# vimalabs/VIMA

Measured on NVIDIA B200. Metric: policy steps/sec (batched action decode), higher is better.
Workload: dtype f16 hi*hi + e4m3 cross terms (2 tensor pass-equivalents), f16 3-term in attention, fp32 accumulate/softmax/LN

## Files before the change

### vima_b200/build.py

```python
from __future__ import annotations

import hashlib
import os
import subprocess
import sys
from concurrent.futures import ThreadPoolExecutor

HERE = os.path.dirname(os.path.abspath(__file__))
CSRC = os.path.join(HERE, "csrc")
OUT_DIR = os.path.join(HERE, "_lib")
LIB_PATH = os.path.join(OUT_DIR, "libvima_b200.so")
SOURCES = ["api.cu", "gemm_tc_f16.cu", "gemm_tc_bf16.cu", "norm.cu", "attention.cu", "attention_tc.cu", "attention_tail.cu", "gemm_simt.cu", "misc.cu", "prepare.cu"]
HEADERS = ["common.cuh", "kernels.h", "gemm_tc.cuh", "gemm_tc_variants.cuh", os.path.join("..", "..", "include", "vima_b200.h")]
NVCC_FLAGS = [
    "-gencode", "arch=compute_100a,code=sm_100a", "-O3", "-lineinfo", "-std=c++17", "--expt-relaxed-constexpr",
    "-Xcompiler", "-fPIC", "-Xcompiler", "-fvisibility=hidden",
]


def _nvcc() -> str:
    for p in (os.environ.get("NVCC"), "/usr/local/cuda/bin/nvcc", "nvcc"):
        if p and (os.path.isfile(p) or p == "nvcc"):
            return p
    raise RuntimeError("nvcc not found")


def _digest() -> str:
    h = hashlib.sha256()
    for f in SOURCES + HEADERS:
        with open(os.path.join(CSRC, f), "rb") as fh:
            h.update(fh.read())
    h.update(" ".join(NVCC_FLAGS).encode())
    return h.hexdigest()


def build(force: bool = False, verbose: bool = False) -> str:
    os.makedirs(OUT_DIR, exist_ok=True)
    stamp = os.path.join(OUT_DIR, "build.sha256")
    dig = _digest()
    if not force and os.path.isfile(LIB_PATH) and os.path.isfile(stamp) and open(stamp).read().strip() == dig:
        return LIB_PATH
    nvcc = _nvcc()

    def compile_one(src: str) -> str:
        obj = os.path.join(OUT_DIR, src.replace(".cu", ".o"))
        cmd = [nvcc, *NVCC_FLAGS, "-c", os.path.join(CSRC, src), "-o", obj]
        if verbose:
            cmd.insert(1, "-Xptxas")
            cmd.insert(2, "-v")
        r = subprocess.run(cmd, capture_output=True, text=True)
        if r.returncode != 0:
            raise RuntimeError(f"nvcc failed for {src}:\n{r.stdout}\n{r.stderr}")
        if verbose:
            print(r.stderr)
        return obj

    with ThreadPoolExecutor(max_workers=len(SOURCES)) as ex:
        objs = list(ex.map(compile_one, SOURCES))
    r = subprocess.run([nvcc, "-shared", "-o", LIB_PATH, *objs, "-cudart", "static"], capture_output=True, text=True)
    if r.returncode != 0:
        raise RuntimeError(f"link failed:\n{r.stdout}\n{r.stderr}")
    with open(stamp, "w") as fh:
        fh.write(dig)
    return LIB_PATH


if __name__ == "__main__":
    print(build(force="--force" in sys.argv, verbose="--verbose" in sys.argv))
```

### vima_b200/csrc/api.cu

```cuda
#include <cstdarg>
#include <cstddef>
#include <cstdio>
#include <cstring>
#include <cstdlib>

#include "../../include/vima_b200.h"
#include "gemm_tc_variants.cuh"
#include "kernels.h"

using namespace vima;

struct vima_ctx {
  int device;
  int sm_count;
  int max_smem_optin;
  long long launches;
  char err[512];
  void* encode_tiled;
  bool gemm_attr_set;
  int attn_tc;
  int attn_tail;
  int gemm_mode;
  int epi_prefetch;
};

struct DeviceGuard {
  int prev = -1;
  bool armed = false;
  cudaError_t enter(int dev) {
    cudaError_t e = cudaGetDevice(&prev);
    if (e != cudaSuccess) return e;
    if (prev == dev) return cudaSuccess;
    armed = true;
    return cudaSetDevice(dev);
  }
  ~DeviceGuard() {
    if (armed) cudaSetDevice(prev);
  }
};

typedef CUresult (*PFN_encodeTiled)(CUtensorMap*, CUtensorMapDataType, cuuint32_t, void*, const cuuint64_t*, const cuuint64_t*,
                                    const cuuint32_t*, const cuuint32_t*, CUtensorMapInterleave, CUtensorMapSwizzle,
                                    CUtensorMapL2promotion, CUtensorMapFloatOOBfill);

static int fail(vima_ctx* c, int code, const char* fmt, ...) {
  if (c) {
    va_list ap;
    va_start(ap, fmt);
    vsnprintf(c->err, sizeof(c->err), fmt, ap);
    va_end(ap);
  }
  return code;
}
static int cuda_fail(vima_ctx* c, cudaError_t e, const char* what) {
  return fail(c, VIMA_E_CUDA, "%s: %s", what, cudaGetErrorString(e));
}
#define CHECK_CTX(c)                  \
  if (!(c)) return VIMA_E_INVALID;    \
  DeviceGuard dev_guard_;             \
  {                                   \
    cudaError_t e_ = dev_guard_.enter((c)->device); \
    if (e_ != cudaSuccess) return cuda_fail((c), e_, "cudaSetDevice"); \
  }

template <class D>
static int load_desc(vima_ctx* c, const D* in, D* out, size_t min_size, const char* what) {
  if (!in) return fail(c, VIMA_E_INVALID, "%s: null descriptor", what);
  const uint32_t sz = in->struct_size;
  if (sz < min_size || sz > sizeof(D))
    return fail(c, VIMA_E_INVALID, "%s: descriptor struct_size %u outside [%zu, %zu] (C-ABI v%d): the caller was built against another vima_b200.h",
                what, sz, min_size, sizeof(D), VIMA_B200_ABI_VERSION);
  memset(out, 0, sizeof(D));
  memcpy(out, in, sz);
  return VIMA_OK;
}
#define LAUNCHED(c, expr, name)                          \
  {                                                      \
    cudaError_t e_ = (expr);                             \
    if (e_ != cudaSuccess) return cuda_fail((c), e_, name); \
    (c)->launches++;                                     \
    return VIMA_OK;                                      \
  }

extern "C" {

int vima_abi_version(void) { return VIMA_B200_ABI_VERSION; }

int vima_set_option(vima_ctx* c, const char* key, const char* value) {
  if (!c) return VIMA_E_INVALID;
  if (!key || !value) return fail(c, VIMA_E_INVALID, "set_option: null key or value");
  if (!strcmp(key, "attn")) {
    if (!strcmp(value, "tc")) { c->attn_tc = 1; return VIMA_OK; }
    if (!strcmp(value, "mma")) { c->attn_tc = 0; return VIMA_OK; }
  } else if (!strcmp(key, "attn_tail")) {
    if (!strcmp(value, "kernel")) { c->attn_tail = 1; return VIMA_OK; }
    if (!strcmp(value, "off")) { c->attn_tail = 0; return VIMA_OK; }
  } else if (!strcmp(key, "gemm_mode")) {
    if (!strcmp(value, "1cta")) { c->gemm_mode = 0; return VIMA_OK; }
    if (!strcmp(value, "mcast")) { c->gemm_mode = 1; return VIMA_OK; }
    if (!strcmp(value, "2cta")) { c->gemm_mode = 2; return VIMA_OK; }
  } else if (!strcmp(key, "epi_prefetch")) {
    if (!strcmp(value, "0") || !strcmp(value, "1")) { c->epi_prefetch = value[0] == '1'; return VIMA_OK; }
  }
  return fail(c, VIMA_E_INVALID, "set_option: unknown option %s=%s", key, value);
}

int vima_create(vima_ctx** out, int device) {
  if (!out) return VIMA_E_INVALID;
  *out = nullptr;
  int n = 0;
  if (cudaGetDeviceCount(&n) != cudaSuccess || device < 0 || device >= n) return VIMA_E_CUDA;
  cudaDeviceProp prop;
  if (cudaGetDeviceProperties(&prop, device) != cudaSuccess) return VIMA_E_CUDA;
  if (prop.major != 10) return VIMA_E_UNSUPPORTED;
  vima_ctx* c = new vima_ctx();
  memset(c, 0, sizeof(*c));
  c->device = device;
  c->sm_count = prop.multiProcessorCount;
  c->max_smem_optin = (int)prop.sharedMemPerBlockOptin;
  DeviceGuard guard;
  if (guard.enter(device) != cudaSuccess) { delete c; return VIMA_E_CUDA; }
  cudaFree(0);
  cudaDriverEntryPointQueryResult q;
  void* fn = nullptr;
  if (cudaGetDriverEntryPoint("cuTensorMapEncodeTiled", &fn, cudaEnableDefault, &q) != cudaSuccess || fn == nullptr) {
    delete c;
    return VIMA_E_CUDA;
  }
  c->encode_tiled = fn;
  c->attn_tc = 1; c->attn_tail = 1; c->gemm_mode = 2; c->epi_prefetch = 0;
  if (const char* e = getenv("VIMA_B200_ATTN")) vima_set_option(c, "attn", e);
  if (const char* e = getenv("VIMA_B200_ATTN_TAIL")) vima_set_option(c, "attn_tail", e);
  if (const char* e = getenv("VIMA_B200_GEMM_MODE")) vima_set_option(c, "gemm_mode", e);
  if (const char* e = getenv("VIMA_B200_EPI_PREFETCH")) vima_set_option(c, "epi_prefetch", e);
  c->err[0] = 0;
  *out = c;
  return VIMA_OK;
}

void vima_destroy(vima_ctx* c) { delete c; }
const char* vima_last_error(vima_ctx* c) { return c ? c->err : "null context"; }
int vima_sm_count(vima_ctx* c) { return c ? c->sm_count : 0; }
int vima_sizeof_gemm_desc(void) { return (int)sizeof(vima_gemm_desc); }
int vima_sizeof_norm_desc(void) { return (int)sizeof(vima_norm_desc); }
int vima_sizeof_attn_desc(void) { return (int)sizeof(vima_attn_desc); }
int vima_sizeof_f32_gemm_group(void) { return (int)sizeof(vima_f32_gemm_group); }
int64_t vima_launch_count(vima_ctx* c) { return c ? c->launches : 0; }

int vima_split_f32(vima_ctx* c, const float* x, int64_t rows, int cols, int ldx, void* hi, void* lo, int ld16, int pad_cols, float scale,
                   int dtype, void* stream) {
  CHECK_CTX(c);
  if (!x || !hi || pad_cols < cols || pad_cols > ld16) return fail(c, VIMA_E_INVALID, "split_f32: bad arguments");
  LAUNCHED(c, launch_split(x, rows, cols, ldx, (unsigned short*)hi, (unsigned short*)lo, ld16, pad_cols, scale, dtype, (cudaStream_t)stream),
           "split_f32");
}

int vima_pack_weight(vima_ctx* c, const float* w, int n, int k, int transposed, int ldw, void* hi, void* lo, int ld16, float scale, int dtype,
                     void* stream) {
  CHECK_CTX(c);
  if (!w || !hi || ld16 < k || (ld16 & 7)) return fail(c, VIMA_E_INVALID, "pack_weight: ld16 must be >= k and a multiple of 8");
  LAUNCHED(c, launch_pack_weight(w, n, k, transposed, ldw, (unsigned short*)hi, (unsigned short*)lo, ld16, scale, dtype, (cudaStream_t)stream),
           "pack_weight");
}

int vima_pack_weight_f8(vima_ctx* c, const float* w, int n, int k, int transposed, int ldw, void* hi8, void* lo8, int ld8, float scale, void* stream) {
  CHECK_CTX(c);
  if (!w || !hi8 || !lo8 || ld8 < k || (ld8 & 15)) return fail(c, VIMA_E_INVALID, "pack_weight_f8: ld8 must be >= k and a multiple of 16");
  LAUNCHED(c, launch_pack_weight_f8(w, n, k, transposed, ldw, (unsigned char*)hi8, (unsigned char*)lo8, ld8, scale, (cudaStream_t)stream),
           "pack_weight_f8");
}

int vima_split_f8(vima_ctx* c, const float* x, int64_t rows, int cols, int ldx, void* lo8, void* hi8, int ld8, void* stream) {
  CHECK_CTX(c);
  if (!x || !lo8 || !hi8 || (cols & 3) || (ldx & 3) || (ld8 & 3) || ld8 < cols) return fail(c, VIMA_E_INVALID, "split_f8: bad arguments");
  LAUNCHED(c, launch_split_f8(x, rows, cols, ldx, (unsigned char*)lo8, (unsigned char*)hi8, ld8, (cudaStream_t)stream), "split_f8");
}

static int choose_block_n(int N, int glu) {
  const int step = glu ? 64 : 32;
  int best = step, best_pad = 1 << 30;
  for (int bn = step; bn <= 256; bn += step) {
    const int padded = ((N + bn - 1) / bn) * bn;
    if (padded < best_pad || (padded == best_pad && bn > best)) { best = bn; best_pad = padded; }
  }
  return best;
}
int vima_glu_block_n(int n_out) { return choose_block_n(2 * n_out, 1); }
int vima_gemm_stats_parts(int N, int glu, int block_n) {
  const int bn = block_n > 0 ? block_n : choose_block_n(N, glu);
  return 2 * ((N + bn - 1) / bn);
}

int vima_row_stats_finalize(vima_ctx* c, const float* partial, int64_t rows, int parts, int cols, float eps, int rms, float* stats, void* stream) {
  CHECK_CTX(c);
  if (!partial || !stats || rows < 0 || parts <= 0 || cols <= 0 || ((uintptr_t)partial & 7) || ((uintptr_t)stats & 7))
    return fail(c, VIMA_E_INVALID, "row_stats_finalize: bad arguments");
  LAUNCHED(c, launch_row_stats_finalize(partial, rows, parts, cols, eps, rms, stats, (cudaStream_t)stream), "row_stats_finalize");
}

static int make_tmap_f8(vima_ctx* c, CUtensorMap* tm, const void* base, int rows, int cols, int ld, int box_rows) {
  const cuuint64_t gdim[2] = {(cuuint64_t)cols, (cuuint64_t)rows};
  const cuuint64_t gstride[1] = {(cuuint64_t)ld};
  const cuuint32_t box[2] = {(cuuint32_t)GEMM_BK, (cuuint32_t)box_rows};
  const cuuint32_t estr[2] = {1, 1};
  CUresult r = ((PFN_encodeTiled)c->encode_tiled)(tm, CU_TENSOR_MAP_DATA_TYPE_UINT8, 2, const_cast<void*>(base), gdim, gstride, box, estr,
                                                  CU_TENSOR_MAP_INTERLEAVE_NONE, CU_TENSOR_MAP_SWIZZLE_64B, CU_TENSOR_MAP_L2_PROMOTION_L2_256B,
                                                  CU_TENSOR_MAP_FLOAT_OOB_FILL_NONE);
  if (r != CUDA_SUCCESS) return fail(c, VIMA_E_CUDA, "cuTensorMapEncodeTiled(fp8) failed (%d): rows %d cols %d ld %d box %d", (int)r, rows, cols, ld, box_rows);
  return VIMA_OK;
}

static int make_tmap(vima_ctx* c, CUtensorMap* tm, const void* base, int dtype, int rows, int cols, int ld, int box_rows) {
  const cuuint64_t gdim[2] = {(cuuint64_t)cols, (cuuint64_t)rows};
  const cuuint64_t gstride[1] = {(cuuint64_t)ld * 2};
  const cuuint32_t box[2] = {(cuuint32_t)GEMM_BK, (cuuint32_t)box_rows};
  const cuuint32_t estr[2] = {1, 1};
  const CUtensorMapDataType dt = dtype == DT_BF16 ? CU_TENSOR_MAP_DATA_TYPE_BFLOAT16 : CU_TENSOR_MAP_DATA_TYPE_FLOAT16;
  CUresult r = ((PFN_encodeTiled)c->encode_tiled)(tm, dt, 2, const_cast<void*>(base), gdim, gstride, box, estr, CU_TENSOR_MAP_INTERLEAVE_NONE,
                                                  CU_TENSOR_MAP_SWIZZLE_128B, CU_TENSOR_MAP_L2_PROMOTION_L2_256B,
                                                  CU_TENSOR_MAP_FLOAT_OOB_FILL_NONE);
  if (r != CUDA_SUCCESS) return fail(c, VIMA_E_CUDA, "cuTensorMapEncodeTiled failed (%d): rows %d cols %d ld %d box %d", (int)r, rows, cols, ld, box_rows);
  return VIMA_OK;
}

int vima_gemm(vima_ctx* c, const vima_gemm_desc* d_in, void* stream) {
  CHECK_CTX(c);
  vima_gemm_desc d_local;
  if (int rc_ = load_desc(c, d_in, &d_local, VIMA_GEMM_DESC_V4_SIZE, "gemm")) return rc_;
  const vima_gemm_desc* d = &d_local;
  if (!d->a_hi || !d->b_hi) return fail(c, VIMA_E_INVALID, "gemm: null operand");
  if (d->M <= 0 || d->N <= 0 || d->K <= 0) return fail(c, VIMA_E_INVALID, "gemm: empty problem");
  if ((d->lda & 7) || (d->ldb & 7) || ((uintptr_t)d->a_hi & 15) || ((uintptr_t)d->b_hi & 15))
    return fail(c, VIMA_E_INVALID, "gemm: operands need 16-byte aligned bases and ld %% 8 == 0 (lda %d ldb %d)", d->lda, d->ldb);
  if ((d->a_lo == nullptr) != (d->b_lo == nullptr)) return fail(c, VIMA_E_INVALID, "gemm: a_lo and b_lo must both be set or both be null");
  const bool f8 = d->a_lo8 || d->a_hi8 || d->b_hi8 || d->b_lo8;
  if (f8) {
    if (!(d->a_lo8 && d->a_hi8 && d->b_hi8 && d->b_lo8) || d->a_lo || d->dtype != DT_F16)
      return fail(c, VIMA_E_INVALID, "gemm: f16f8 mode needs all four e4m3 operands, fp16 hi operands and no 16-bit lo operands");
    if ((d->lda8 & 15) || (d->ldb8 & 15) || ((uintptr_t)d->a_lo8 & 15) || ((uintptr_t)d->a_hi8 & 15) || ((uintptr_t)d->b_hi8 & 15) ||
        ((uintptr_t)d->b_lo8 & 15) || d->lda8 < d->K || d->ldb8 < d->K)
      return fail(c, VIMA_E_INVALID, "gemm: e4m3 operands need 16-byte aligned bases and ld %% 16 == 0");
  }
  if ((d->out_lo8 == nullptr) != (d->out_hi8 == nullptr) || (d->out_lo8 && (!d->out_hi || d->dtype != DT_F16 || (d->ld_o8 & 3))))
    return fail(c, VIMA_E_INVALID, "gemm: out_lo8/out_hi8 come together, with an fp16 out_hi, ld_o8 %% 4 == 0");
  if (d->lda < d->K || d->ldb < d->K) return fail(c, VIMA_E_INVALID, "gemm: leading dimension smaller than K");
  int bn = d->block_n > 0 ? d->block_n : choose_block_n(d->N, d->glu);
  if (bn > 256 || (bn % (d->glu ? 64 : 32))) return fail(c, VIMA_E_INVALID, "gemm: bad block_n %d", bn);
  if (d->glu && (d->N % bn)) return fail(c, VIMA_E_INVALID, "gemm: GLU needs N %% block_n == 0");
  {
    const int n_out = d->glu ? d->N / 2 : d->N;
    const bool bad = (n_out & 3) || (d->out_f32 && ((d->ld_o32 & 3) || ((uintptr_t)d->out_f32 & 15))) ||
                     (d->out_hi && ((d->ld_o16 & 3) || ((uintptr_t)d->out_hi & 7) || (d->out_lo && ((uintptr_t)d->out_lo & 7)))) ||
                     (d->mul && ((d->ld_mul & 3) || ((uintptr_t)d->mul & 15))) || (d->residual && ((d->ld_res & 3) || ((uintptr_t)d->residual & 15)));
    if (bad) return fail(c, VIMA_E_INVALID, "gemm: epilogue tensors need N %% 4 == 0, ld %% 4 == 0 and 16-byte (fp32) / 8-byte (16-bit) aligned bases");
  }

  if (d->row_stats) {
    if (!d->ln_c1 || (d->ln_cols != 1 && d->ln_cols != 2) || (d->ln_cols == 2 && !d->glu) || ((uintptr_t)d->row_stats & 7))
      return fail(c, VIMA_E_INVALID, "gemm: folded LayerNorm needs row_stats (8-byte aligned), ln_c1 and ln_cols 1 (all columns) or 2 (GLU value half)");
  }
  if (d->res_stats) {
    if (!d->residual || !d->res_gamma || !d->res_beta || d->glu || ((uintptr_t)d->res_stats & 7))
      return fail(c, VIMA_E_INVALID, "gemm: a LayerNorm'd residual needs residual, res_stats (8-byte aligned), res_gamma, res_beta and no GLU");
  }
  if (d->stats_out) {
    if (d->stats_parts != 2 * ((d->N + bn - 1) / bn) || ((uintptr_t)d->stats_out & 7))
      return fail(c, VIMA_E_INVALID, "gemm: stats_parts must be vima_gemm_stats_parts(N, glu, block_n) = %d (got %d)", 2 * ((d->N + bn - 1) / bn), d->stats_parts);
  }

  GemmParams p;
  memset(&p, 0, sizeof(p));
  const int split = f8 ? 2 : (d->a_lo != nullptr ? 1 : 0);
  int rc;
  const int tiles_m_ = (d->M + GEMM_BM - 1) / GEMM_BM, tiles_n_ = (d->N + bn - 1) / bn;
  const int mode_pref = c->gemm_mode;
  const bool pair_ok = (bn % 64) == 0 && ((tiles_m_ + 1) / 2) * tiles_n_ >= c->sm_count / 2 && tiles_m_ >= 2;
  const int mcast = (pair_ok && mode_pref == 1) ? 1 : 0;
  const int two_cta = (pair_ok && mode_pref == 2) ? 1 : 0;
  const int b_box = (mcast || two_cta) ? bn / 2 : bn;
  if ((rc = make_tmap(c, &p.tm_a_hi, d->a_hi, d->dtype, d->M, d->K, d->lda, GEMM_BM))) return rc;
  if ((rc = make_tmap(c, &p.tm_b_hi, d->b_hi, d->dtype, d->N, d->K, d->ldb, b_box))) return rc;
  if (split == 1) {
    if ((rc = make_tmap(c, &p.tm_a_lo, d->a_lo, d->dtype, d->M, d->K, d->lda, GEMM_BM))) return rc;
    if ((rc = make_tmap(c, &p.tm_b_lo, d->b_lo, d->dtype, d->N, d->K, d->ldb, b_box))) return rc;
  } else if (split == 2) {
    if ((rc = make_tmap_f8(c, &p.tm_a_lo, d->a_lo8, d->M, d->K, d->lda8, GEMM_BM))) return rc;
    if ((rc = make_tmap_f8(c, &p.tm_a_hi8, d->a_hi8, d->M, d->K, d->lda8, GEMM_BM))) return rc;
    if ((rc = make_tmap_f8(c, &p.tm_b_hi8, d->b_hi8, d->N, d->K, d->ldb8, b_box))) return rc;
    if ((rc = make_tmap_f8(c, &p.tm_b_lo, d->b_lo8, d->N, d->K, d->ldb8, b_box))) return rc;
  }
  p.M = d->M; p.N = d->N; p.K = d->K;
  p.block_n = bn;
  p.mcast = mcast;
  p.two_cta = two_cta;
  p.split = split;
  p.dtype = d->dtype;
  p.glu = d->glu;
  p.epi_prefetch = c->epi_prefetch;
  p.act = d->act;
  p.acc_scale = d->acc_scale == 0.f ? 1.f : d->acc_scale;
  p.bias = d->bias;
  p.mul = d->mul; p.ld_mul = d->ld_mul;
  p.residual = d->residual; p.ld_res = d->ld_res;
  p.out_f32 = d->out_f32; p.ld_o32 = d->ld_o32;
  p.out_hi = (unsigned short*)d->out_hi; p.out_lo = (unsigned short*)d->out_lo; p.ld_o16 = d->ld_o16;
  p.out_lo8 = (unsigned char*)d->out_lo8; p.out_hi8 = (unsigned char*)d->out_hi8; p.ld_o8 = d->ld_o8;
  p.row_stats = d->row_stats; p.ln_c1 = d->ln_c1; p.ln_cols = d->ln_cols;
  p.res_stats = d->res_stats; p.res_gamma = d->res_gamma; p.res_beta = d->res_beta;
  p.stats_out = d->stats_out; p.stats_parts = d->stats_parts;

  const size_t stage = (size_t)(GEMM_A_TILE_BYTES + (two_cta ? bn / 2 : bn) * 128) * (split ? 2 : 1);
  const size_t fixed = gemm_smem_bytes(bn, split, 0, two_cta);
  int n_stages = (int)(((size_t)c->max_smem_optin - fixed) / stage);
  if (n_stages > GEMM_MAX_STAGES) n_stages = GEMM_MAX_STAGES;
  if (n_stages < 2) return fail(c, VIMA_E_UNSUPPORTED, "gemm: not enough shared memory for 2 stages");
  p.n_stages = n_stages;
  const size_t smem = gemm_smem_bytes(bn, split, n_stages, two_cta);
  const int tiles = mcast ? ((tiles_m_ + 1) / 2) * tiles_n_ : tiles_m_ * tiles_n_;
  int grid = tiles < c->sm_count ? tiles : c->sm_count;
  if (mcast || two_cta) grid = 2 * (tiles < c->sm_count / 2 ? tiles : c->sm_count / 2);
  GemmLaunch l;
  l.act = d->act; l.glu = d->glu != 0; l.mul = d->mul != nullptr; l.res = d->residual != nullptr;
  l.o32 = d->out_f32 != nullptr; l.o16 = d->out_hi != nullptr; l.dtype = d->dtype;
  l.lna = d->row_stats != nullptr; l.lnr = d->res_stats != nullptr; l.stats = d->stats_out != nullptr; l.device = c->device;
  if (d->dtype == DT_BF16) { LAUNCHED(c, launch_gemm_tc_bf16(p, l, grid, smem, c->max_smem_optin, (cudaStream_t)stream), "gemm_tc_kernel"); }
  LAUNCHED(c, launch_gemm_tc_f16(p, l, grid, smem, c->max_smem_optin, (cudaStream_t)stream), "gemm_tc_kernel");
}

int vima_gemm_f32_grouped(vima_ctx* c, const vima_f32_gemm_group* groups_dev, int n_groups, int M, int max_n, int act, void* stream) {
  CHECK_CTX(c);
  static_assert(sizeof(vima_f32_gemm_group) == sizeof(SimtGemmGroup), "group layout");
  if (!groups_dev) return fail(c, VIMA_E_INVALID, "gemm_f32_grouped: null groups");
  LAUNCHED(c, launch_simt_gemm_grouped(reinterpret_cast<const SimtGemmGroup*>(groups_dev), n_groups, M, max_n, act, (cudaStream_t)stream),
           "simt_gemm");
}

int vima_gemm_f32_grouped_host(vima_ctx* c, const vima_f32_gemm_group* groups_host, int n_groups, int M, int max_n, int act, void* stream) {
  CHECK_CTX(c);
  if (!groups_host || n_groups < 0) return fail(c, VIMA_E_INVALID, "gemm_f32_grouped_host: null groups");
  cudaError_t e = launch_simt_gemm_grouped_host(reinterpret_cast<const SimtGemmGroup*>(groups_host), n_groups, M, max_n, act, (cudaStream_t)stream);
  if (e != cudaSuccess) return cuda_fail(c, e, "simt_gemm");
  c->launches += (n_groups + SIMT_MAX_HOST_GROUPS - 1) / SIMT_MAX_HOST_GROUPS;
  return VIMA_OK;
}

int vima_norm(vima_ctx* c, const vima_norm_desc* d_in, void* stream) {
  CHECK_CTX(c);
  vima_norm_desc d_local;
  if (int rc_ = load_desc(c, d_in, &d_local, VIMA_NORM_DESC_V4_SIZE, "norm")) return rc_;
  const vima_norm_desc* d = &d_local;
  if (!d->x) return fail(c, VIMA_E_INVALID, "norm: null input");
  if ((d->cols & 3) || d->cols > 1024 || d->cols <= 0) return fail(c, VIMA_E_INVALID, "norm: cols must be a multiple of 4, <= 1024 (got %d)", d->cols);
  if ((d->ldx & 3) || (d->add && (d->ld_add & 3)) || (d->out_f32 && (d->ld_o32 & 3)) || (d->out2_f32 && (d->ld_o2 & 3)) || (d->out_hi && (d->ld_o16 & 3)))
    return fail(c, VIMA_E_INVALID, "norm: leading dimensions must be multiples of 4");
  NormParams p;
  p.x = d->x; p.rows = d->rows; p.cols = d->cols; p.ldx = d->ldx;
  p.add = d->add; p.ld_add = d->ld_add;
  p.w = d->w; p.b = d->b; p.eps = d->eps; p.rms = d->rms;
  p.w2 = d->w2; p.b2 = d->b2; p.eps2 = d->eps2;
  p.out_f32 = d->out_f32; p.ld_o32 = d->ld_o32;
  p.out2_f32 = d->out2_f32; p.ld_o2 = d->ld_o2;
  p.out_hi = (unsigned short*)d->out_hi; p.out_lo = (unsigned short*)d->out_lo; p.ld_o16 = d->ld_o16;
  p.dtype = d->dtype;
  p.out_lo8 = (unsigned char*)d->out_lo8; p.out_hi8 = (unsigned char*)d->out_hi8; p.ld_o8 = d->ld_o8;
  p.stats_out = d->stats_out; p.stats_eps = d->stats_eps;
  if (p.stats_out && ((uintptr_t)p.stats_out & 7)) return fail(c, VIMA_E_INVALID, "norm: stats_out must be 8-byte aligned");
  if ((p.out_lo8 == nullptr) != (p.out_hi8 == nullptr) || (p.out_lo8 && (p.ld_o8 & 3)))
    return fail(c, VIMA_E_INVALID, "norm: out_lo8/out_hi8 come together with ld_o8 %% 4 == 0");
  LAUNCHED(c, launch_norm(p, (cudaStream_t)stream), "norm");
}

int vima_attention(vima_ctx* c, const vima_attn_desc* d_in, void* stream) {
  CHECK_CTX(c);
  vima_attn_desc d_local;
  if (int rc_ = load_desc(c, d_in, &d_local, VIMA_ATTN_DESC_V4_SIZE, "attention")) return rc_;
  const vima_attn_desc* d = &d_local;
  if (!d->q_hi || !d->k_hi || !d->v_hi || !d->o_hi) return fail(c, VIMA_E_INVALID, "attention: null operand");
  if (d->D != 32 && d->D != 64) return fail(c, VIMA_E_UNSUPPORTED, "attention: head_dim %d (32 and 64 are built)", d->D);
  if ((d->ldq & 7) || (d->ldk & 7) || (d->ldv & 7) || (d->ldo & 1)) return fail(c, VIMA_E_INVALID, "attention: leading dimensions must be multiples of 8");
  const bool split = d->q_lo != nullptr;
  if (split != (d->k_lo != nullptr) || split != (d->v_lo != nullptr)) return fail(c, VIMA_E_INVALID, "attention: q/k/v lo parts must be all set or all null");
  if (d->rel_bias && d->Lq != d->Lk) return fail(c, VIMA_E_INVALID, "attention: relative bias needs Lq == Lk");
  if (!(d->scale > 0.f)) return fail(c, VIMA_E_INVALID, "attention: scale must be positive");
  AttnParams p;
  p.q_hi = (const unsigned short*)d->q_hi; p.q_lo = (const unsigned short*)d->q_lo; p.ldq = d->ldq;
  p.k_hi = (const unsigned short*)d->k_hi; p.k_lo = (const unsigned short*)d->k_lo; p.ldk = d->ldk;
  p.v_hi = (const unsigned short*)d->v_hi; p.v_lo = (const unsigned short*)d->v_lo; p.ldv = d->ldv;
  p.key_mask = d->key_mask; p.rel_bias = d->rel_bias;
  p.o_hi = (unsigned short*)d->o_hi; p.o_lo = (unsigned short*)d->o_lo; p.ldo = d->ldo;
  p.B = d->B; p.H = d->H; p.Lq = d->Lq; p.Lk = d->Lk; p.D = d->D;
  p.scale = d->scale; p.causal = d->causal; p.split = split; p.dtype = d->dtype;
  p.o_lo8 = (unsigned char*)d->o_lo8; p.o_hi8 = (unsigned char*)d->o_hi8; p.ldo8 = d->ldo8;
  p.kv_batch_rows = d->kv_batch_rows; p.mask_ld = d->mask_ld; p.q_pos0 = d->q_pos0; p.q_batch_rows = 0;
  if ((d->kv_batch_rows && d->kv_batch_rows < d->Lk) || (d->mask_ld && d->mask_ld < d->Lk) || d->q_pos0 < 0)
    return fail(c, VIMA_E_INVALID, "attention: kv_batch_rows / mask_ld must cover Lk, q_pos0 >= 0");
  if ((p.o_lo8 == nullptr) != (p.o_hi8 == nullptr) || (p.o_lo8 && ((p.ldo8 & 1) || d->dtype != DT_F16)))
    return fail(c, VIMA_E_INVALID, "attention: o_lo8/o_hi8 come together (fp16 format, even ldo8)");
  if (c->attn_tc && attention_tc_supported(p)) {
    const int tail = p.Lq % 128;
    if (c->attn_tail && p.Lq > 128 && tail >= 1 && tail <= ATTN_TAIL_MAX_ROWS) {
      AttnParams body = p;
      body.Lq = p.Lq - tail;
      body.q_batch_rows = p.Lq;
      cudaError_t e_ = launch_attention_tc(body, c->encode_tiled, (cudaStream_t)stream);
      if (e_ != cudaSuccess) return cuda_fail(c, e_, "attention_tc");
      c->launches++;
      LAUNCHED(c, launch_attention_tail(p, p.Lq - tail, tail, (cudaStream_t)stream), "attention_tail");
    }
    LAUNCHED(c, launch_attention_tc(p, c->encode_tiled, (cudaStream_t)stream), "attention_tc");
  }
  {
    const size_t need = attention_smem_bytes(p);
    if (need > (size_t)c->max_smem_optin)
      return fail(c, VIMA_E_UNSUPPORTED,
                  "attention: Lk = %d keys of head_dim %d (%s operands%s) need %zu bytes of shared memory, the device offers %d: the "
                  "resident-K/V kernel takes Lk <= %d at this head_dim", d->Lk, d->D, split ? "split" : "single", d->rel_bias ? ", relative bias" : "",
                  need, c->max_smem_optin, attention_max_lk(p, (size_t)c->max_smem_optin));
  }
  LAUNCHED(c, launch_attention(p, (cudaStream_t)stream), "attention");
}

int vima_latent_attention(vima_ctx* c, const float* q, int ldq, int64_t q_batch_stride, const float* k, int ldk, const float* v, int ldv, float* o,
                          int ldo, int64_t N, int Lq, int Lk, int H, int d, float scale, void* stream) {
  CHECK_CTX(c);
  if (!q || !k || !v || !o) return fail(c, VIMA_E_INVALID, "latent_attention: null pointer");
  if (Lk < 1 || Lk > 16 || d < 1 || d > 128 || Lq < 0 || N < 0 || H < 1)
    return fail(c, VIMA_E_UNSUPPORTED, "latent_attention: 1..16 keys, head_dim <= 128 (Lk %d, d %d)", Lk, d);
  LatentAttnParams p;
  p.q = q; p.ldq = ldq; p.q_batch_stride = q_batch_stride; p.k = k; p.ldk = ldk; p.v = v; p.ldv = ldv; p.o = o; p.ldo = ldo;
  p.N = N; p.Lq = Lq; p.Lk = Lk; p.H = H; p.d = d; p.scale = scale;
  LAUNCHED(c, launch_latent_attention(p, (cudaStream_t)stream), "latent_attention");
}

int vima_small_attention(vima_ctx* c, const float* qkv, int ld, int64_t N, int S, int H, int W, float scale, void* o_hi, void* o_lo, int ldo,
                         float* o_f32, int dtype, void* stream) {
  CHECK_CTX(c);
  if (!qkv) return fail(c, VIMA_E_INVALID, "small_attention: null input");
  SmallAttnParams p;
  p.qkv = qkv; p.ld = ld; p.o_hi = (unsigned short*)o_hi; p.o_lo = (unsigned short*)o_lo; p.ldo = ldo; p.o_f32 = o_f32;
  p.N = N; p.S = S; p.H = H; p.W = W; p.scale = scale; p.dtype = dtype;
  LAUNCHED(c, launch_small_attention(p, (cudaStream_t)stream), "small_attention");
}

int vima_assemble_history(vima_ctx* c, const float* obs, const uint8_t* obs_mask, const float* action, int T, int B, int Q, int E, int La,
                          float* tokens, uint8_t* masks_bl, int64_t* pos_bl, void* stream) {
  CHECK_CTX(c);
  if (!obs || !obs_mask || !tokens || !masks_bl || !pos_bl || (La > 0 && !action) || (E & 3))
    return fail(c, VIMA_E_INVALID, "assemble_history: bad arguments");
  if (La != T && La != T - 1) return fail(c, VIMA_E_INVALID, "assemble_history: need T-1 or T action tokens");
  cudaError_t e = launch_assemble_history(obs, obs_mask, action, T, B, Q, E, La, tokens, masks_bl, (long long*)pos_bl, (cudaStream_t)stream);
  if (e != cudaSuccess) return cuda_fail(c, e, "assemble_history");
  c->launches += 2;
  return VIMA_OK;
}

int vima_mask_cumsum(vima_ctx* c, const uint8_t* mask, int B, int L, int64_t* pos, void* stream) {
  CHECK_CTX(c);
  LAUNCHED(c, launch_mask_cumsum(mask, B, L, (long long*)pos, (cudaStream_t)stream), "mask_cumsum");
}

int vima_add_pos_embed(vima_ctx* c, const float* tok, int64_t stride_b, int64_t stride_l, const int64_t* ids, const float* table, int n_pos, int B,
                       int L, int E, float* out_f32, void* hi, void* lo, int ld16, int dtype, int* err_flag, void* stream) {
  CHECK_CTX(c);
  if ((E & 3) || (stride_b & 3) || (stride_l & 3) || (hi && (ld16 & 3))) return fail(c, VIMA_E_INVALID, "add_pos_embed: alignment");
  LAUNCHED(c, launch_add_pos_embed(tok, stride_b, stride_l, (const long long*)ids, table, n_pos, B, L, E, out_f32, (unsigned short*)hi,
                                   (unsigned short*)lo, ld16, dtype, err_flag, (cudaStream_t)stream),
           "add_pos_embed");
}

int vima_gather_prompt(vima_ctx* c, const int32_t* kind, const int32_t* index, const int64_t* word_ids, const float* word_table,
                       const float* img_emb, const uint8_t* img_mask, int B, int Lp, int D, float* out, uint8_t* mask_out, void* stream) {
  CHECK_CTX(c);
  if (D & 3) return fail(c, VIMA_E_INVALID, "gather_prompt: D %% 4");
  LAUNCHED(c, launch_gather_prompt(kind, index, (const long long*)word_ids, word_table, img_emb, img_mask, B, Lp, D, out, mask_out,
                                   (cudaStream_t)stream),
           "gather_prompt");
}

int vima_patchify(vima_ctx* c, const uint8_t* img, int64_t N, int H, int W, int P, void* hi, void* lo, int ld16, int dtype, void* stream) {
  CHECK_CTX(c);
  if ((P & 3) || (H % P) || (W % P) || (ld16 & 3) || ld16 < 3 * P * P) return fail(c, VIMA_E_INVALID, "patchify: bad geometry");
  LAUNCHED(c, launch_patchify(img, N, H, W, P, (unsigned short*)hi, (unsigned short*)lo, ld16, dtype, (cudaStream_t)stream), "patchify");
}

int vima_vit_tokens(vima_ctx* c, const float* patch_out, const float* cls, const float* pos, int64_t N, int S, int W, float* out, void* stream) {
  CHECK_CTX(c);
  if (W & 3) return fail(c, VIMA_E_INVALID, "vit_tokens: W %% 4");
  LAUNCHED(c, launch_vit_tokens(patch_out, cls, pos, N, S, W, out, (cudaStream_t)stream), "vit_tokens");
}

int vima_bbox_norm(vima_ctx* c, const int64_t* bbox, int64_t n, float* out, void* stream) {
  CHECK_CTX(c);
  LAUNCHED(c, launch_bbox_norm((const long long*)bbox, n, out, (cudaStream_t)stream), "bbox_norm");
}

int vima_fill_ee(vima_ctx* c, const int64_t* ee, const float* table, int64_t n_te, int Q, void* hi, void* lo, int ld16, int col0, int n_pad,
                 int dtype, void* stream) {
  CHECK_CTX(c);
  LAUNCHED(c, launch_fill_ee((const long long*)ee, table, n_te, Q, (unsigned short*)hi, (unsigned short*)lo, ld16, col0, n_pad, dtype,
                             (cudaStream_t)stream),
           "fill_ee");
}

int vima_gato_positions(vima_ctx* c, const uint8_t* prompt_mask, int B, int Lp, int L, uint8_t* mask_out, int64_t* pos_out, void* stream) {
  CHECK_CTX(c);
  if (!prompt_mask || !mask_out || !pos_out || L < Lp) return fail(c, VIMA_E_INVALID, "gato_positions: bad arguments");
  LAUNCHED(c, launch_gato_positions(prompt_mask, B, Lp, L, mask_out, (long long*)pos_out, (cudaStream_t)stream), "gato_positions");
}

int vima_max_u8(vima_ctx* c, const uint8_t* x, int64_t n, int* out_max, void* stream) {
  CHECK_CTX(c);
  LAUNCHED(c, launch_max_u8(x, n, out_max, (cudaStream_t)stream), "max_u8");
}

int vima_action_scale(vima_ctx* c, const int64_t* idx, int64_t n, int width, const float* bins_dev, float* out, void* stream) {
  CHECK_CTX(c);
  LAUNCHED(c, launch_action_scale((const long long*)idx, n, width, bins_dev, out, (cudaStream_t)stream), "action_scale");
}

int vima_object_stats(vima_ctx* c, const void* segm, int segm_elem_bytes, int n_img, int H, int W, const int64_t* obj_ids_dev, int n_obj,
                      int ids_per_image, int32_t* stats, void* stream) {
  CHECK_CTX(c);
  if ((segm_elem_bytes != 1 && segm_elem_bytes != 4 && segm_elem_bytes != 8) || n_obj < 0 || n_obj > 64 || n_img < 0 || H <= 0 || W <= 0)
    return fail(c, VIMA_E_INVALID, "object_stats: segm elements of 1/4/8 bytes, at most 64 object ids per image");
  LAUNCHED(c, launch_object_stats(segm, segm_elem_bytes, n_img, H, W, (const long long*)obj_ids_dev, n_obj, ids_per_image, stats,
                                  (cudaStream_t)stream), "object_stats");
}

int vima_crop_resize(vima_ctx* c, const uint8_t* rgb, int n_img, int H, int W, const int32_t* stats, int n_obj, uint8_t* crops,
                     int64_t* bbox, uint8_t* mask, int32_t* n_valid, void* stream) {
  CHECK_CTX(c);
  if (n_obj < 0 || n_obj > 64 || n_img < 0 || n_img > 65535 || H <= 0 || W <= 0)
    return fail(c, VIMA_E_INVALID, "crop_resize: at most 64 object ids per image and 65535 images per call");
  LAUNCHED(c, launch_crop_resize(rgb, n_img, H, W, stats, n_obj, crops, (long long*)bbox, mask, n_valid, (cudaStream_t)stream),
           "crop_resize");
}

int vima_action_postprocess(vima_ctx* c, const int64_t* idx, int64_t n, int width, const float* bins_dev, const float* lo_dev,
                            const float* hi_dev, int bound_stride, float* out, void* stream) {
  CHECK_CTX(c);
  if (width <= 0 || n < 0 || (bound_stride != 0 && bound_stride < width))
    return fail(c, VIMA_E_INVALID, "action_postprocess: width > 0, n >= 0, bound_stride 0 (broadcast) or >= width");
  LAUNCHED(c, launch_action_post((const long long*)idx, n, width, bins_dev, lo_dev, hi_dev, bound_stride, out, (cudaStream_t)stream),
           "action_postprocess");
}

int vima_head_select(vima_ctx* c, const float* logits, int B, int n_heads, const int32_t* head_off_dev, float* logits_norm, int64_t* modes,
                     void* stream) {
  CHECK_CTX(c);
  LAUNCHED(c, launch_head_select(logits, B, n_heads, head_off_dev, logits_norm, (long long*)modes, (cudaStream_t)stream), "head_select");
}

}
```

### vima_b200/csrc/attention.cu

```cuda
#include "kernels.h"

namespace vima {

constexpr float FP32_MIN = -3.4028234663852886e38f;
constexpr float LOG2E = 1.4426950408889634f;

template <int DT>
__device__ __forceinline__ void mma16816(float (&c)[4], const uint32_t (&a)[4], uint32_t b0, uint32_t b1) {
  if constexpr (DT == DT_F16) {
    asm volatile("mma.sync.aligned.m16n8k16.row.col.f32.f16.f16.f32 {%0,%1,%2,%3}, {%4,%5,%6,%7}, {%8,%9}, {%0,%1,%2,%3};"
                 : "+f"(c[0]), "+f"(c[1]), "+f"(c[2]), "+f"(c[3])
                 : "r"(a[0]), "r"(a[1]), "r"(a[2]), "r"(a[3]), "r"(b0), "r"(b1));
  } else {
    asm volatile("mma.sync.aligned.m16n8k16.row.col.f32.bf16.bf16.f32 {%0,%1,%2,%3}, {%4,%5,%6,%7}, {%8,%9}, {%0,%1,%2,%3};"
                 : "+f"(c[0]), "+f"(c[1]), "+f"(c[2]), "+f"(c[3])
                 : "r"(a[0]), "r"(a[1]), "r"(a[2]), "r"(a[3]), "r"(b0), "r"(b1));
  }
}

template <int DT>
__device__ __forceinline__ void pack_split(float x0, float x1, uint32_t& hi, uint32_t& lo) { split2<DT>(x0, x1, hi, lo); }

__device__ __forceinline__ void ldmatrix_x4(uint32_t (&r)[4], const void* smem_row_ptr) {
  asm volatile("ldmatrix.sync.aligned.m8n8.x4.shared.b16 {%0,%1,%2,%3}, [%4];"
               : "=r"(r[0]), "=r"(r[1]), "=r"(r[2]), "=r"(r[3])
               : "r"(smem_u32(smem_row_ptr)));
}

constexpr float CAUSAL_L2 = -1e4f * LOG2E;
constexpr float EXIT_L2 = -9000.f * LOG2E;

template <int D, int DT, bool SPLIT>
__global__ void __launch_bounds__(256, (D == 32) ? 2 : 1) attention_kernel(const AttnParams p) {
  constexpr int KS = D / 16;
  constexpr int ND = D / 8;
  constexpr int KROW = D + 8;
  extern __shared__ __align__(16) unsigned char smem[];
  const int h = blockIdx.x, b = blockIdx.y;
  const int Lk = p.Lk, Lq = p.Lq;
  const int Lk_pad = (Lk + 63) & ~63;
  const int VROW = Lk_pad + 8;
  const int n_kt = Lk_pad / 64;
  unsigned short* Ks_hi = reinterpret_cast<unsigned short*>(smem);
  unsigned short* Ks_lo = Ks_hi + (SPLIT ? Lk_pad * KROW : 0);
  unsigned short* Vt_hi = Ks_lo + Lk_pad * KROW;
  unsigned short* Vt_lo = Vt_hi + (SPLIT ? D * VROW : 0);
  float* maskadd = reinterpret_cast<float*>(Vt_lo + D * VROW);
  int* tile_plain = reinterpret_cast<int*>(maskadd + Lk_pad);
  int* qb_counter = tile_plain + n_kt;
  float* sbias = reinterpret_cast<float*>(qb_counter + 1);

  const int tid = threadIdx.x, lane = tid & 31, warp = tid >> 5;
  const int kvb = p.kv_batch_rows ? p.kv_batch_rows : Lk;
  const int mld = p.mask_ld ? p.mask_ld : Lk;
  const int qp0 = p.q_pos0;
  const int qbr = p.q_batch_rows ? p.q_batch_rows : Lq;
  constexpr int CH = D / 8;
  for (int idx = tid; idx < Lk_pad * CH; idx += 256) {
    const int j = idx / CH, c = idx % CH;
    uint4 kh = make_uint4(0, 0, 0, 0), kl = kh, vh = kh, vl = kh;
    if (j < Lk) {
      const size_t rk = ((size_t)b * kvb + j) * p.ldk + h * D + c * 8;
      const size_t rv = ((size_t)b * kvb + j) * p.ldv + h * D + c * 8;
      kh = __ldg(reinterpret_cast<const uint4*>(p.k_hi + rk));
      vh = __ldg(reinterpret_cast<const uint4*>(p.v_hi + rv));
      if (SPLIT) {
        kl = __ldg(reinterpret_cast<const uint4*>(p.k_lo + rk));
        vl = __ldg(reinterpret_cast<const uint4*>(p.v_lo + rv));
      }
    }
    *reinterpret_cast<uint4*>(Ks_hi + j * KROW + c * 8) = kh;
    if (SPLIT) *reinterpret_cast<uint4*>(Ks_lo + j * KROW + c * 8) = kl;
    const unsigned short* vhs = reinterpret_cast<const unsigned short*>(&vh);
    const unsigned short* vls = reinterpret_cast<const unsigned short*>(&vl);
#pragma unroll
    for (int e = 0; e < 8; ++e) {
      Vt_hi[(c * 8 + e) * VROW + j] = vhs[e];
      if (SPLIT) Vt_lo[(c * 8 + e) * VROW + j] = vls[e];
    }
  }
  for (int j = tid; j < Lk_pad; j += 256) {
    float m = -INFINITY;
    if (j < Lk) m = (p.key_mask == nullptr || p.key_mask[(size_t)b * mld + j]) ? 0.f : FP32_MIN;
    maskadd[j] = m;
  }
  if (p.rel_bias)
    for (int j = tid; j < 2 * Lk - 1; j += 256) sbias[j] = __ldg(p.rel_bias + (size_t)h * (2 * Lk - 1) + j) * LOG2E;
  if (tid == 0) *qb_counter = 0;
  __syncthreads();
  for (int kt = warp; kt < n_kt; kt += 8) {
    const bool ok = (maskadd[kt * 64 + lane] == 0.f) && (maskadd[kt * 64 + 32 + lane] == 0.f);
    const bool all_ok = __all_sync(0xffffffffu, ok);
    if (lane == 0) tile_plain[kt] = all_ok ? 1 : 0;
  }
  __syncthreads();

  const int g = lane >> 2, t = lane & 3;
  const int n_qb = (Lq + 15) / 16;
  const float c_l2 = p.scale * LOG2E;
  const int lm_row = lane & 7, lm_chunk = (lane >> 3) * 8;
  for (;;) {
    int ticket = 0;
    if (lane == 0) ticket = atomicAdd(qb_counter, 1);
    ticket = __shfl_sync(0xffffffffu, ticket, 0);
    if (ticket >= n_qb) break;
    const int qb = n_qb - 1 - ticket;
    const int r0 = qb * 16 + g, r1 = r0 + 8;
    uint32_t qh[KS][4], ql[KS][4];
#pragma unroll
    for (int ks = 0; ks < KS; ++ks) {
#pragma unroll
      for (int e = 0; e < 4; ++e) {
        const int r = (e & 1) ? r1 : r0;
        const int c = ks * 16 + 2 * t + ((e & 2) ? 8 : 0);
        uint32_t vh = 0, vl = 0;
        if (r < Lq) {
          const size_t off = ((size_t)b * qbr + r) * p.ldq + h * D + c;
          vh = __ldg(reinterpret_cast<const uint32_t*>(p.q_hi + off));
          if (SPLIT) vl = __ldg(reinterpret_cast<const uint32_t*>(p.q_lo + off));
        }
        qh[ks][e] = vh;
        ql[ks][e] = vl;
      }
    }
    float o[ND][4];
#pragma unroll
    for (int n = 0; n < ND; ++n) o[n][0] = o[n][1] = o[n][2] = o[n][3] = 0.f;
    float mrow[2] = {-INFINITY, -INFINITY}, lrow[2] = {0.f, 0.f};

    for (int kt = 0; kt < n_kt; ++kt) {
      float s[8][4];
#pragma unroll
      for (int nt = 0; nt < 8; ++nt) s[nt][0] = s[nt][1] = s[nt][2] = s[nt][3] = 0.f;
#pragma unroll
      for (int half = 0; half < 2; ++half) {
#pragma unroll
        for (int kk = 0; kk < KS; kk += 2) {
          uint32_t bh[4][4], bl[4][4];
#pragma unroll
          for (int q = 0; q < 4; ++q) {
            const int key = kt * 64 + (half * 4 + q) * 8 + lm_row;
            ldmatrix_x4(bh[q], Ks_hi + key * KROW + kk * 16 + lm_chunk);
            if (SPLIT) ldmatrix_x4(bl[q], Ks_lo + key * KROW + kk * 16 + lm_chunk);
          }
#pragma unroll
          for (int k2 = 0; k2 < 2; ++k2) {
#pragma unroll
            for (int q = 0; q < 4; ++q) mma16816<DT>(s[half * 4 + q], qh[kk + k2], bh[q][2 * k2], bh[q][2 * k2 + 1]);
            if (SPLIT) {
#pragma unroll
              for (int q = 0; q < 4; ++q) mma16816<DT>(s[half * 4 + q], ql[kk + k2], bh[q][2 * k2], bh[q][2 * k2 + 1]);
#pragma unroll
              for (int q = 0; q < 4; ++q) mma16816<DT>(s[half * 4 + q], qh[kk + k2], bl[q][2 * k2], bl[q][2 * k2 + 1]);
            }
          }
        }
      }
      const bool needs_mask = !tile_plain[kt];
      const bool needs_causal = p.causal && (kt * 64 + 63 > qb * 16 + qp0);
      float mx[2] = {-INFINITY, -INFINITY};
      if (!needs_mask && !needs_causal && p.rel_bias == nullptr) {
#pragma unroll
        for (int nt = 0; nt < 8; ++nt) {
#pragma unroll
          for (int e = 0; e < 4; ++e) {
            const float y = s[nt][e] * c_l2;
            s[nt][e] = y;
            mx[e >> 1] = fmaxf(mx[e >> 1], y);
          }
        }
      } else {
#pragma unroll
        for (int nt = 0; nt < 8; ++nt) {
#pragma unroll
          for (int e = 0; e < 4; ++e) {
            const int j = kt * 64 + nt * 8 + 2 * t + (e & 1);
            const int i = (e & 2) ? r1 : r0;
            float y = s[nt][e] * c_l2;
            if (p.rel_bias && j < Lk) y += sbias[j - min(i, Lq - 1) + Lk - 1];
            if (needs_causal && j > i + qp0) y = CAUSAL_L2;
            if (needs_mask) y += maskadd[j];
            s[nt][e] = y;
            mx[e >> 1] = fmaxf(mx[e >> 1], y);
          }
        }
      }
      float corr[2];
#pragma unroll
      for (int r = 0; r < 2; ++r) {
        mx[r] = fmaxf(mx[r], __shfl_xor_sync(0xffffffffu, mx[r], 1));
        mx[r] = fmaxf(mx[r], __shfl_xor_sync(0xffffffffu, mx[r], 2));
        const float m_new = fmaxf(mrow[r], mx[r]);
        corr[r] = ex2_approx(mrow[r] - m_new);
        mrow[r] = m_new;
        lrow[r] *= corr[r];
      }
      float ps[2] = {0.f, 0.f};
#pragma unroll
      for (int nt = 0; nt < 8; ++nt) {
#pragma unroll
        for (int e = 0; e < 4; ++e) {
          const float pv = ex2_approx(s[nt][e] - mrow[e >> 1]);
          s[nt][e] = pv;
          ps[e >> 1] += pv;
        }
      }
      lrow[0] += ps[0];
      lrow[1] += ps[1];
#pragma unroll
      for (int n = 0; n < ND; ++n) {
        o[n][0] *= corr[0]; o[n][1] *= corr[0];
        o[n][2] *= corr[1]; o[n][3] *= corr[1];
      }
      uint32_t ph[4][4], pl[4][4];
#pragma unroll
      for (int k2 = 0; k2 < 4; ++k2) {
        pack_split<DT>(s[2 * k2][0], s[2 * k2][1], ph[k2][0], pl[k2][0]);
        pack_split<DT>(s[2 * k2][2], s[2 * k2][3], ph[k2][1], pl[k2][1]);
        pack_split<DT>(s[2 * k2 + 1][0], s[2 * k2 + 1][1], ph[k2][2], pl[k2][2]);
        pack_split<DT>(s[2 * k2 + 1][2], s[2 * k2 + 1][3], ph[k2][3], pl[k2][3]);
      }
#pragma unroll
      for (int ng = 0; ng < ND; ng += 4) {
#pragma unroll
        for (int kp = 0; kp < 2; ++kp) {
          uint32_t vh4[4][4], vl4[4][4];
#pragma unroll
          for (int q = 0; q < 4; ++q) {
            const int drow = (ng + q) * 8 + lm_row;
            ldmatrix_x4(vh4[q], Vt_hi + drow * VROW + kt * 64 + kp * 32 + lm_chunk);
            if (SPLIT) ldmatrix_x4(vl4[q], Vt_lo + drow * VROW + kt * 64 + kp * 32 + lm_chunk);
          }
#pragma unroll
          for (int k2 = 0; k2 < 2; ++k2) {
#pragma unroll
            for (int q = 0; q < 4; ++q) mma16816<DT>(o[ng + q], ph[2 * kp + k2], vh4[q][2 * k2], vh4[q][2 * k2 + 1]);
            if (SPLIT) {
#pragma unroll
              for (int q = 0; q < 4; ++q) mma16816<DT>(o[ng + q], pl[2 * kp + k2], vh4[q][2 * k2], vh4[q][2 * k2 + 1]);
#pragma unroll
              for (int q = 0; q < 4; ++q) mma16816<DT>(o[ng + q], ph[2 * kp + k2], vl4[q][2 * k2], vl4[q][2 * k2 + 1]);
            }
          }
        }
      }
      if (p.causal && (kt + 1) * 64 > qb * 16 + 15 + qp0) {
        const bool done = (mrow[0] > EXIT_L2) && (mrow[1] > EXIT_L2);
        if (__all_sync(0xffffffffu, done)) break;
      }
    }
#pragma unroll
    for (int r = 0; r < 2; ++r) {
      lrow[r] += __shfl_xor_sync(0xffffffffu, lrow[r], 1);
      lrow[r] += __shfl_xor_sync(0xffffffffu, lrow[r], 2);
    }
    const float inv0 = 1.0f / lrow[0], inv1 = 1.0f / lrow[1];
#pragma unroll
    for (int n = 0; n < ND; ++n) {
      const int c = h * D + n * 8 + 2 * t;
      uint32_t hi, lo;
#pragma unroll
      for (int half = 0; half < 2; ++half) {
        const int r = half ? r1 : r0;
        if (r >= Lq) continue;
        const float x0 = o[n][2 * half] * (half ? inv1 : inv0), x1 = o[n][2 * half + 1] * (half ? inv1 : inv0);
        pack_split<DT>(x0, x1, hi, lo);
        const size_t off = ((size_t)b * qbr + r) * p.ldo + c;
        *reinterpret_cast<uint32_t*>(p.o_hi + off) = hi;
        if (p.o_lo) *reinterpret_cast<uint32_t*>(p.o_lo + off) = lo;
        if (p.o_lo8) {
          const float2 hf = __half22float2(*reinterpret_cast<const __half2*>(&hi));
          unsigned short l8, h8;
          asm("cvt.rn.satfinite.e4m3x2.f32 %0, %1, %2;" : "=h"(l8) : "f"((x1 - hf.y) * F8_ACT_LO_SCALE), "f"((x0 - hf.x) * F8_ACT_LO_SCALE));
          asm("cvt.rn.satfinite.e4m3x2.f32 %0, %1, %2;" : "=h"(h8) : "f"(x1 * F8_ACT_HI_SCALE), "f"(x0 * F8_ACT_HI_SCALE));
          const size_t off8 = ((size_t)b * qbr + r) * p.ldo8 + c;
          *reinterpret_cast<unsigned short*>(p.o_lo8 + off8) = l8;
          *reinterpret_cast<unsigned short*>(p.o_hi8 + off8) = h8;
        }
      }
    }
  }
}

size_t attention_smem_bytes(const AttnParams& p) {
  const int D = p.D;
  const int Lk_pad = (p.Lk + 63) & ~63;
  const size_t parts = p.split ? 2 : 1;
  size_t smem = parts * (size_t)Lk_pad * (D + 8) * 2 + parts * (size_t)D * (Lk_pad + 8) * 2 + (size_t)Lk_pad * 4 + (size_t)(Lk_pad / 64 + 1) * 4;
  if (p.rel_bias) smem += (size_t)(2 * p.Lk) * 4;
  return smem;
}

int attention_max_lk(const AttnParams& p, size_t smem_limit) {
  AttnParams q = p;
  int best = 0;
  for (int lk = 64; lk <= 4096; lk += 64) {
    q.Lk = lk;
    if (attention_smem_bytes(q) <= smem_limit) best = lk; else break;
  }
  return best;
}

template <int D, int DT, bool SPLIT>
static cudaError_t launch_attn_t(const AttnParams& p, cudaStream_t stream) {
  const size_t smem = attention_smem_bytes(p);
  auto kern = attention_kernel<D, DT, SPLIT>;
  static int attr_smem[64] = {};
  int dev = 0;
  cudaGetDevice(&dev);
  if ((int)smem > attr_smem[dev & 63]) {
    cudaError_t e = cudaFuncSetAttribute(kern, cudaFuncAttributeMaxDynamicSharedMemorySize, (int)smem);
    if (e != cudaSuccess) return e;
    attr_smem[dev & 63] = (int)smem;
  }
  dim3 grid(p.H, p.B);
  kern<<<grid, 256, smem, stream>>>(p);
  return cudaGetLastError();
}

cudaError_t launch_attention(const AttnParams& p, cudaStream_t stream) {
  if (p.B == 0 || p.Lq == 0) return cudaSuccess;
  const bool sp = p.split != 0;
  if (p.D == 32) {
    if (p.dtype == DT_F16) return sp ? launch_attn_t<32, DT_F16, true>(p, stream) : launch_attn_t<32, DT_F16, false>(p, stream);
    return sp ? launch_attn_t<32, DT_BF16, true>(p, stream) : launch_attn_t<32, DT_BF16, false>(p, stream);
  }
  if (p.D == 64) {
    if (p.dtype == DT_F16) return sp ? launch_attn_t<64, DT_F16, true>(p, stream) : launch_attn_t<64, DT_F16, false>(p, stream);
    return sp ? launch_attn_t<64, DT_BF16, true>(p, stream) : launch_attn_t<64, DT_BF16, false>(p, stream);
  }
  return cudaErrorInvalidValue;
}

constexpr int SMALL_S_MAX = 16;

template <int DT>
__global__ void __launch_bounds__(128) small_attention_kernel(const SmallAttnParams p) {
  const long long t = (long long)blockIdx.x * blockDim.x + threadIdx.x;
  const int S = p.S;
  if (t >= p.N * p.H * S) return;
  const int i = (int)(t % S);
  const long long nh = t / S;
  const int h = (int)(nh % p.H);
  const long long n = nh / p.H;
  const float* base = p.qkv + (size_t)(n * S) * p.ld + h * 32;
  float4 q[8];
#pragma unroll
  for (int c = 0; c < 8; ++c) q[c] = __ldg(reinterpret_cast<const float4*>(base + (size_t)i * p.ld) + c);
  float sc[SMALL_S_MAX];
  float mx = -INFINITY;
#pragma unroll
  for (int j = 0; j < SMALL_S_MAX; ++j) {
    if (j < S) {
      const float4* kr = reinterpret_cast<const float4*>(base + (size_t)j * p.ld + p.W);
      float a0 = 0.f, a1 = 0.f;
#pragma unroll
      for (int c = 0; c < 8; c += 2) {
        const float4 k0 = __ldg(kr + c), k1 = __ldg(kr + c + 1);
        a0 = fmaf(q[c].x, k0.x, a0); a0 = fmaf(q[c].y, k0.y, a0); a0 = fmaf(q[c].z, k0.z, a0); a0 = fmaf(q[c].w, k0.w, a0);
        a1 = fmaf(q[c + 1].x, k1.x, a1); a1 = fmaf(q[c + 1].y, k1.y, a1); a1 = fmaf(q[c + 1].z, k1.z, a1); a1 = fmaf(q[c + 1].w, k1.w, a1);
      }
      sc[j] = (a0 + a1) * p.scale;
      mx = fmaxf(mx, sc[j]);
    }
  }
  float den = 0.f;
#pragma unroll
  for (int j = 0; j < SMALL_S_MAX; ++j) {
    if (j < S) {
      sc[j] = expf(sc[j] - mx);
      den += sc[j];
    }
  }
  const float inv = 1.0f / den;
  float4 o[8];
#pragma unroll
  for (int c = 0; c < 8; ++c) o[c] = make_float4(0.f, 0.f, 0.f, 0.f);
#pragma unroll
  for (int j = 0; j < SMALL_S_MAX; ++j) {
    if (j < S) {
      const float4* vr = reinterpret_cast<const float4*>(base + (size_t)j * p.ld + 2 * p.W);
      const float w = sc[j] * inv;
#pragma unroll
      for (int c = 0; c < 8; ++c) {
        const float4 v = __ldg(vr + c);
        o[c].x = fmaf(w, v.x, o[c].x); o[c].y = fmaf(w, v.y, o[c].y); o[c].z = fmaf(w, v.z, o[c].z); o[c].w = fmaf(w, v.w, o[c].w);
      }
    }
  }
  const size_t off = (size_t)(n * S + i) * p.ldo + h * 32;
#pragma unroll
  for (int c = 0; c < 8; ++c) {
    if (p.o_f32) *reinterpret_cast<float4*>(p.o_f32 + off + c * 4) = o[c];
    if (p.o_hi) {
      uint2 hi, lo;
      split4v<DT>(o[c], hi, lo);
      *reinterpret_cast<uint2*>(p.o_hi + off + c * 4) = hi;
      if (p.o_lo) *reinterpret_cast<uint2*>(p.o_lo + off + c * 4) = lo;
    }
  }
}

cudaError_t launch_small_attention(const SmallAttnParams& p, cudaStream_t stream) {
  if (p.N == 0) return cudaSuccess;
  if (p.S > SMALL_S_MAX || p.S < 1 || p.W != p.H * 32 || (p.ld & 3) || (p.ldo & 3)) return cudaErrorInvalidValue;
  const long long threads = p.N * p.H * p.S;
  const long long blocks = (threads + 127) / 128;
  if (p.dtype == DT_BF16)
    small_attention_kernel<DT_BF16><<<(unsigned)blocks, 128, 0, stream>>>(p);
  else
    small_attention_kernel<DT_F16><<<(unsigned)blocks, 128, 0, stream>>>(p);
  return cudaGetLastError();
}

constexpr int LAT_LK_MAX = 16, LAT_DV = 4;

__global__ void __launch_bounds__(256) latent_attention_kernel(const LatentAttnParams p) {
  const long long w = ((long long)blockIdx.x * blockDim.x + threadIdx.x) >> 5;
  const int lane = threadIdx.x & 31;
  if (w >= p.N * p.H) return;
  const long long n = w / p.H;
  const int h = (int)(w % p.H);
  const int d = p.d;
  const float* qb = p.q + (size_t)n * p.q_batch_stride + h * d;
  const float* kb = p.k + (size_t)n * p.Lk * p.ldk + h * d;
  const float* vb = p.v + (size_t)n * p.Lk * p.ldv + h * d;
  for (int i = 0; i < p.Lq; ++i) {
    float qv[LAT_DV];
#pragma unroll
    for (int e = 0; e < LAT_DV; ++e) qv[e] = (lane + 32 * e < d) ? __ldg(qb + (size_t)i * p.ldq + lane + 32 * e) : 0.f;
    float sc[LAT_LK_MAX];
    float mx = -INFINITY;
#pragma unroll
    for (int j = 0; j < LAT_LK_MAX; ++j) {
      if (j < p.Lk) {
        float part = 0.f;
#pragma unroll
        for (int e = 0; e < LAT_DV; ++e)
          if (lane + 32 * e < d) part = fmaf(qv[e], __ldg(kb + (size_t)j * p.ldk + lane + 32 * e), part);
        sc[j] = warp_sum(part) * p.scale;
        mx = fmaxf(mx, sc[j]);
      }
    }
    float den = 0.f, acc[LAT_DV] = {0.f, 0.f, 0.f, 0.f};
#pragma unroll
    for (int j = 0; j < LAT_LK_MAX; ++j) {
      if (j < p.Lk) {
        const float e_ = expf(sc[j] - mx);
        den += e_;
#pragma unroll
        for (int e = 0; e < LAT_DV; ++e)
          if (lane + 32 * e < d) acc[e] = fmaf(e_, __ldg(vb + (size_t)j * p.ldv + lane + 32 * e), acc[e]);
      }
    }
    const float inv = 1.0f / den;
#pragma unroll
    for (int e = 0; e < LAT_DV; ++e)
      if (lane + 32 * e < d) p.o[((size_t)n * p.Lq + i) * p.ldo + h * d + lane + 32 * e] = acc[e] * inv;
  }
}

cudaError_t launch_latent_attention(const LatentAttnParams& p, cudaStream_t stream) {
  if (p.N == 0 || p.Lq == 0) return cudaSuccess;
  if (p.Lk > LAT_LK_MAX || p.Lk < 1 || p.d > 32 * LAT_DV || p.d < 1) return cudaErrorInvalidValue;
  const long long warps = p.N * p.H;
  latent_attention_kernel<<<(unsigned)((warps + 7) / 8), 256, 0, stream>>>(p);
  return cudaGetLastError();
}

}
```

### vima_b200/csrc/attention_tail.cu

```cuda
#include "kernels.h"

namespace vima {

namespace {

constexpr int TAIL_NT = ATTN_TAIL_MAX_ROWS;
constexpr int TAIL_WARPS = 8;
constexpr int TAIL_D = 32;
constexpr float FP32_MIN_TL = -3.4028234663852886e38f;
constexpr float LOG2E_TL = 1.4426950408889634f;
constexpr float CAUSAL_L2_TL = -1e4f * LOG2E_TL;

template <int DT>
__device__ __forceinline__ float2 unpack2(uint32_t w) {
  if constexpr (DT == DT_F16) return __half22float2(*reinterpret_cast<const __half2*>(&w));
  else return __bfloat1622float2(*reinterpret_cast<const __nv_bfloat162*>(&w));
}
__device__ __forceinline__ unsigned long long pack2(float x, float y) {
  unsigned long long r;
  asm("mov.b64 %0, {%1, %2};" : "=l"(r) : "f"(x), "f"(y));
  return r;
}
__device__ __forceinline__ float2 unpack64(unsigned long long v) {
  float2 r;
  asm("mov.b64 {%0, %1}, %2;" : "=f"(r.x), "=f"(r.y) : "l"(v));
  return r;
}
__device__ __forceinline__ void ffma2(unsigned long long& acc, unsigned long long a, unsigned long long b) {
  asm("fma.rn.f32x2 %0, %1, %2, %0;" : "+l"(acc) : "l"(a), "l"(b));
}

template <int DT>
__global__ void __launch_bounds__(TAIL_WARPS * 32) attention_tail_kernel(const AttnParams p, int row0, int nt, int lk_pad) {
  extern __shared__ __align__(16) float smt[];
  const int warp = threadIdx.x >> 5, lane = threadIdx.x & 31;
  const long long unit = (long long)blockIdx.x * TAIL_WARPS + warp;
  if (unit >= (long long)p.B * p.H) return;
  const int b = (int)(unit / p.H), h = (int)(unit % p.H);
  const int Lk = p.Lk;
  const int kvb = p.kv_batch_rows ? p.kv_batch_rows : Lk;
  const int mld = p.mask_ld ? p.mask_ld : Lk;
  const int qbr = p.q_batch_rows ? p.q_batch_rows : p.Lq;
  float* qs = smt + (size_t)warp * (TAIL_NT * TAIL_D + (size_t)lk_pad * TAIL_NT);
  float* sc = qs + TAIL_NT * TAIL_D;

  const float c_l2 = p.scale * LOG2E_TL;
#pragma unroll
  for (int i = 0; i < TAIL_NT; ++i) {
    float q = 0.f;
    if (i < nt) {
      const size_t off = ((size_t)b * qbr + row0 + i) * p.ldq + h * TAIL_D + lane;
      q = Op16<DT>::back(p.q_hi[off]);
      if (p.q_lo) q += Op16<DT>::back(p.q_lo[off]);
    }
    qs[i * TAIL_D + lane] = q * c_l2;
  }
  __syncwarp();

  float mx[TAIL_NT];
#pragma unroll
  for (int i = 0; i < TAIL_NT; ++i) mx[i] = -INFINITY;
  const int pos0 = row0 + p.q_pos0;
  uint4 kh[4], kl[4];
  auto load_k = [&](int j) {
#pragma unroll
    for (int c = 0; c < 4; ++c) { kh[c] = make_uint4(0u, 0u, 0u, 0u); kl[c] = kh[c]; }
    if (j < Lk) {
      const size_t rk = ((size_t)b * kvb + j) * p.ldk + h * TAIL_D;
      const uint4* ph = reinterpret_cast<const uint4*>(p.k_hi + rk);
#pragma unroll
      for (int c = 0; c < 4; ++c) kh[c] = __ldg(ph + c);
      if (p.k_lo) {
        const uint4* pl = reinterpret_cast<const uint4*>(p.k_lo + rk);
#pragma unroll
        for (int c = 0; c < 4; ++c) kl[c] = __ldg(pl + c);
      }
    }
  };
  load_k(lane);
  for (int j0 = 0; j0 < lk_pad; j0 += 32) {
    const int j = j0 + lane;
    const bool valid = j < Lk;
    unsigned long long kf[TAIL_D / 2];
#pragma unroll
    for (int c = 0; c < 4; ++c) {
      const uint32_t aw[4] = {kh[c].x, kh[c].y, kh[c].z, kh[c].w};
      const uint32_t lw[4] = {kl[c].x, kl[c].y, kl[c].z, kl[c].w};
#pragma unroll
      for (int e = 0; e < 4; ++e) {
        const float2 x = unpack2<DT>(aw[e]), y = unpack2<DT>(lw[e]);
        kf[c * 4 + e] = pack2(x.x + y.x, x.y + y.y);
      }
    }
    if (j0 + 32 < lk_pad) load_k(j + 32);
    float madd = -INFINITY;
    if (valid) madd = (p.key_mask == nullptr || p.key_mask[(size_t)b * mld + j]) ? 0.f : FP32_MIN_TL;
    float y[TAIL_NT];
#pragma unroll
    for (int i = 0; i < TAIL_NT; ++i) {
      const ulonglong2* q2 = reinterpret_cast<const ulonglong2*>(qs + i * TAIL_D);
      unsigned long long a0 = 0ull, a1 = 0ull;
#pragma unroll
      for (int c = 0; c < TAIL_D / 4; ++c) {
        const ulonglong2 q = q2[c];
        ffma2(a0, q.x, kf[2 * c]);
        ffma2(a1, q.y, kf[2 * c + 1]);
      }
      const float2 s0 = unpack64(a0), s1 = unpack64(a1);
      float v = ((s0.x + s0.y) + (s1.x + s1.y)) + madd;
      if (p.causal && j > pos0 + i) v = CAUSAL_L2_TL + madd;
      y[i] = v;
      mx[i] = fmaxf(mx[i], v);
    }
    float4* dst = reinterpret_cast<float4*>(sc + (size_t)j * TAIL_NT);
    dst[0] = make_float4(y[0], y[1], y[2], y[3]);
    dst[1] = make_float4(y[4], y[5], y[6], y[7]);
  }
#pragma unroll
  for (int i = 0; i < TAIL_NT; ++i) mx[i] = warp_max(mx[i]);

  float ls[TAIL_NT];
#pragma unroll
  for (int i = 0; i < TAIL_NT; ++i) ls[i] = 0.f;
  for (int j0 = 0; j0 < lk_pad; j0 += 32) {
    float4* cell = reinterpret_cast<float4*>(sc + (size_t)(j0 + lane) * TAIL_NT);
    const float4 a = cell[0], c = cell[1];
    float w[TAIL_NT] = {a.x, a.y, a.z, a.w, c.x, c.y, c.z, c.w};
#pragma unroll
    for (int i = 0; i < TAIL_NT; ++i) {
      w[i] = ex2_approx(w[i] - mx[i]);
      ls[i] += w[i];
    }
    cell[0] = make_float4(w[0], w[1], w[2], w[3]);
    cell[1] = make_float4(w[4], w[5], w[6], w[7]);
  }
#pragma unroll
  for (int i = 0; i < TAIL_NT; ++i) ls[i] = warp_sum(ls[i]);
  __syncwarp();

  const int kg = lane >> 3, dg = lane & 7;
  unsigned long long acc[TAIL_NT][2];
#pragma unroll
  for (int i = 0; i < TAIL_NT; ++i) { acc[i][0] = 0ull; acc[i][1] = 0ull; }
  for (int j = kg; j < Lk; j += 16) {
    uint2 vh[4], vl[4];
#pragma unroll
    for (int u = 0; u < 4; ++u) {
      const int jj = j + 4 * u;
      vh[u] = make_uint2(0u, 0u); vl[u] = vh[u];
      if (jj < Lk) {
        const size_t rv = ((size_t)b * kvb + jj) * p.ldv + h * TAIL_D + dg * 4;
        vh[u] = __ldg(reinterpret_cast<const uint2*>(p.v_hi + rv));
        if (p.v_lo) vl[u] = __ldg(reinterpret_cast<const uint2*>(p.v_lo + rv));
      }
    }
#pragma unroll
    for (int u = 0; u < 4; ++u) {
      const int jj = j + 4 * u;
      if (jj >= Lk) break;
      const float2 h0 = unpack2<DT>(vh[u].x), l0 = unpack2<DT>(vl[u].x), h1 = unpack2<DT>(vh[u].y), l1 = unpack2<DT>(vl[u].y);
      const unsigned long long v01 = pack2(h0.x + l0.x, h0.y + l0.y), v23 = pack2(h1.x + l1.x, h1.y + l1.y);
      const float4* cell = reinterpret_cast<const float4*>(sc + (size_t)jj * TAIL_NT);
      const float4 a = cell[0], c = cell[1];
      const float w[TAIL_NT] = {a.x, a.y, a.z, a.w, c.x, c.y, c.z, c.w};
#pragma unroll
      for (int i = 0; i < TAIL_NT; ++i) {
        const unsigned long long ww = pack2(w[i], w[i]);
        ffma2(acc[i][0], ww, v01);
        ffma2(acc[i][1], ww, v23);
      }
    }
  }
#pragma unroll
  for (int i = 0; i < TAIL_NT; ++i) {
    const float2 a01 = unpack64(acc[i][0]), a23 = unpack64(acc[i][1]);
    float4 o = make_float4(a01.x, a01.y, a23.x, a23.y);
    o.x += __shfl_xor_sync(0xffffffffu, o.x, 8); o.y += __shfl_xor_sync(0xffffffffu, o.y, 8);
    o.z += __shfl_xor_sync(0xffffffffu, o.z, 8); o.w += __shfl_xor_sync(0xffffffffu, o.w, 8);
    o.x += __shfl_xor_sync(0xffffffffu, o.x, 16); o.y += __shfl_xor_sync(0xffffffffu, o.y, 16);
    o.z += __shfl_xor_sync(0xffffffffu, o.z, 16); o.w += __shfl_xor_sync(0xffffffffu, o.w, 16);
    if ((i & 3) != kg || i >= nt) continue;
    const float inv = 1.0f / ls[i];
    o.x *= inv; o.y *= inv; o.z *= inv; o.w *= inv;
    const size_t row = (size_t)b * qbr + row0 + i;
    const size_t off = row * p.ldo + h * TAIL_D + dg * 4;
    if (p.o_lo8) {
      uint2 h16;
      uint32_t l8, h8;
      split4_f8(o, F8_ACT_LO_SCALE, F8_ACT_HI_SCALE, h16, l8, h8);
      *reinterpret_cast<uint2*>(p.o_hi + off) = h16;
      const size_t off8 = row * p.ldo8 + h * TAIL_D + dg * 4;
      *reinterpret_cast<uint32_t*>(p.o_lo8 + off8) = l8;
      *reinterpret_cast<uint32_t*>(p.o_hi8 + off8) = h8;
      if (p.o_lo) {
        uint2 hi, lo;
        split4v<DT>(o, hi, lo);
        *reinterpret_cast<uint2*>(p.o_lo + off) = lo;
      }
    } else {
      uint2 hi, lo;
      split4v<DT>(o, hi, lo);
      *reinterpret_cast<uint2*>(p.o_hi + off) = hi;
      if (p.o_lo) *reinterpret_cast<uint2*>(p.o_lo + off) = lo;
    }
  }
}

}

cudaError_t launch_attention_tail(const AttnParams& p, int row0, int nt, cudaStream_t stream) {
  if (p.B == 0 || nt <= 0) return cudaSuccess;
  if (nt > TAIL_NT || p.D != TAIL_D) return cudaErrorInvalidValue;
  const int lk_pad = (p.Lk + 31) & ~31;
  const size_t smem = (size_t)TAIL_WARPS * (TAIL_NT * TAIL_D + (size_t)lk_pad * TAIL_NT) * sizeof(float);
  constexpr size_t smem_max = (size_t)TAIL_WARPS * (TAIL_NT * TAIL_D + 512 * TAIL_NT) * sizeof(float);
  if (smem > smem_max) return cudaErrorInvalidValue;
  static bool attr_set[2][64] = {};
  int dev = 0;
  cudaGetDevice(&dev);
  const int fi = p.dtype == DT_BF16 ? 1 : 0;
  if (!attr_set[fi][dev & 63]) {
    cudaError_t e = fi ? cudaFuncSetAttribute(attention_tail_kernel<DT_BF16>, cudaFuncAttributeMaxDynamicSharedMemorySize, (int)smem_max)
                       : cudaFuncSetAttribute(attention_tail_kernel<DT_F16>, cudaFuncAttributeMaxDynamicSharedMemorySize, (int)smem_max);
    if (e != cudaSuccess) return e;
    attr_set[fi][dev & 63] = true;
  }
  const long long units = (long long)p.B * p.H;
  const unsigned grid = (unsigned)((units + TAIL_WARPS - 1) / TAIL_WARPS);
  if (fi) attention_tail_kernel<DT_BF16><<<grid, TAIL_WARPS * 32, smem, stream>>>(p, row0, nt, lk_pad);
  else attention_tail_kernel<DT_F16><<<grid, TAIL_WARPS * 32, smem, stream>>>(p, row0, nt, lk_pad);
  return cudaGetLastError();
}

}
```

### vima_b200/csrc/attention_tc.cu

```cuda
#include "kernels.h"

namespace vima {

namespace {

constexpr float FP32_MIN_TC = -3.4028234663852886e38f;
constexpr float LOG2E_TC = 1.4426950408889634f;
constexpr float CAUSAL_L2_TC = -1e4f * LOG2E_TC;
constexpr float EXIT_L2_TC = -9000.f * LOG2E_TC;
constexpr float LAZY_THRESH = 8.0f;

constexpr int ATC_THREADS = 160;
constexpr int ATC_BM = 128, ATC_KC = 64, ATC_D = 32;
constexpr int ATC_TMEM_COLS = 128;
constexpr int ATC_MAX_LK = 512;
constexpr int OFF_QH = 0, OFF_QL = 8192;
constexpr int OFF_K = 16384;
constexpr int OFF_VH = 32768, OFF_VL = 36864;
constexpr int OFF_PH = 40960, OFF_PL = 57344;
constexpr int OFF_MASK = 73728;
constexpr int OFF_FLAG = OFF_MASK + ATC_MAX_LK * 4;
constexpr int OFF_BAR = OFF_FLAG + 32;
constexpr int OFF_TPTR = OFF_BAR + 64;
constexpr int ATC_SMEM = OFF_TPTR + 16;

struct AttnTcParams {
  AttnParams a;
  CUtensorMap tm_q_hi, tm_q_lo, tm_k_hi, tm_k_lo, tm_v_hi, tm_v_lo;
};

__device__ __forceinline__ uint64_t desc_sw64(uint32_t a) {
  return (uint64_t)((a >> 4) & 0x3FFF) | (1ull << 16) | ((uint64_t)(512 >> 4) << 32) | (1ull << 46) | (4ull << 61);
}
__device__ __forceinline__ uint64_t desc_sw128(uint32_t a) {
  return (uint64_t)((a >> 4) & 0x3FFF) | (1ull << 16) | ((uint64_t)(1024 >> 4) << 32) | (1ull << 46) | (2ull << 61);
}

__device__ __forceinline__ float max3(float a, float b, float c) {
  float r;
  asm("max.f32 %0, %1, %2, %3;" : "=f"(r) : "f"(a), "f"(b), "f"(c));
  return r;
}
__device__ __forceinline__ void fma2(float& x0, float& x1, float s, float n) {
  unsigned long long xx, ss, nn;
  asm("mov.b64 %0, {%1, %2};" : "=l"(xx) : "f"(x0), "f"(x1));
  asm("mov.b64 %0, {%1, %1};" : "=l"(ss) : "f"(s));
  asm("mov.b64 %0, {%1, %1};" : "=l"(nn) : "f"(n));
  asm("fma.rn.f32x2 %0, %1, %2, %3;" : "=l"(xx) : "l"(xx), "l"(ss), "l"(nn));
  asm("mov.b64 {%0, %1}, %2;" : "=f"(x0), "=f"(x1) : "l"(xx));
}

__device__ __forceinline__ void fma2v(float& x0, float& x1, float s, float n0, float n1) {
  unsigned long long xx, ss, nn;
  asm("mov.b64 %0, {%1, %2};" : "=l"(xx) : "f"(x0), "f"(x1));
  asm("mov.b64 %0, {%1, %1};" : "=l"(ss) : "f"(s));
  asm("mov.b64 %0, {%1, %2};" : "=l"(nn) : "f"(n0), "f"(n1));
  asm("fma.rn.f32x2 %0, %1, %2, %3;" : "=l"(xx) : "l"(xx), "l"(ss), "l"(nn));
  asm("mov.b64 {%0, %1}, %2;" : "=f"(x0), "=f"(x1) : "l"(xx));
}

__device__ __forceinline__ void tmem_st_32x32(uint32_t taddr, const uint32_t (&v)[32]) {
  asm volatile(
      "tcgen05.st.sync.aligned.32x32b.x32.b32 [%0], "
      "{%1, %2, %3, %4, %5, %6, %7, %8, %9, %10, %11, %12, %13, %14, %15, %16, "
      "%17, %18, %19, %20, %21, %22, %23, %24, %25, %26, %27, %28, %29, %30, %31, %32};" ::"r"(taddr),
      "r"(v[0]), "r"(v[1]), "r"(v[2]), "r"(v[3]), "r"(v[4]), "r"(v[5]), "r"(v[6]), "r"(v[7]), "r"(v[8]), "r"(v[9]), "r"(v[10]), "r"(v[11]),
      "r"(v[12]), "r"(v[13]), "r"(v[14]), "r"(v[15]), "r"(v[16]), "r"(v[17]), "r"(v[18]), "r"(v[19]), "r"(v[20]), "r"(v[21]), "r"(v[22]),
      "r"(v[23]), "r"(v[24]), "r"(v[25]), "r"(v[26]), "r"(v[27]), "r"(v[28]), "r"(v[29]), "r"(v[30]), "r"(v[31])
      : "memory");
}
__device__ __forceinline__ void tmem_st_wait() { asm volatile("tcgen05.wait::st.sync.aligned;" ::: "memory"); }

template <int DT>
__device__ __forceinline__ void store_row(const AttnParams& p, int b, int row, int h, const uint32_t (&o)[ATC_D], float inv) {
  const size_t brow = (size_t)b * (p.q_batch_rows ? p.q_batch_rows : p.Lq) + row;
  const size_t off = brow * p.ldo + h * ATC_D;
#pragma unroll
  for (int c8 = 0; c8 < ATC_D / 8; ++c8) {
    uint32_t hi[4], lo[4];
    float x[8];
#pragma unroll
    for (int e = 0; e < 8; ++e) x[e] = __uint_as_float(o[c8 * 8 + e]) * inv;
#pragma unroll
    for (int e = 0; e < 4; ++e) split2<DT>(x[2 * e], x[2 * e + 1], hi[e], lo[e]);
    *reinterpret_cast<uint4*>(p.o_hi + off + c8 * 8) = make_uint4(hi[0], hi[1], hi[2], hi[3]);
    if (p.o_lo) *reinterpret_cast<uint4*>(p.o_lo + off + c8 * 8) = make_uint4(lo[0], lo[1], lo[2], lo[3]);
    if (p.o_lo8) {
      const size_t off8 = brow * p.ldo8 + h * ATC_D + c8 * 8;
      uint32_t l8[2], h8[2];
#pragma unroll
      for (int e = 0; e < 2; ++e) {
        const float2 f01 = __half22float2(*reinterpret_cast<const __half2*>(&hi[2 * e]));
        const float2 f23 = __half22float2(*reinterpret_cast<const __half2*>(&hi[2 * e + 1]));
        l8[e] = e4m3x4((x[4 * e] - f01.x) * F8_ACT_LO_SCALE, (x[4 * e + 1] - f01.y) * F8_ACT_LO_SCALE,
                       (x[4 * e + 2] - f23.x) * F8_ACT_LO_SCALE, (x[4 * e + 3] - f23.y) * F8_ACT_LO_SCALE);
        h8[e] = e4m3x4(x[4 * e] * F8_ACT_HI_SCALE, x[4 * e + 1] * F8_ACT_HI_SCALE, x[4 * e + 2] * F8_ACT_HI_SCALE, x[4 * e + 3] * F8_ACT_HI_SCALE);
      }
      *reinterpret_cast<uint2*>(p.o_lo8 + off8) = make_uint2(l8[0], l8[1]);
      *reinterpret_cast<uint2*>(p.o_hi8 + off8) = make_uint2(h8[0], h8[1]);
    }
  }
}

template <int DT>
__global__ void __launch_bounds__(ATC_THREADS, 3) attention_tc_kernel(const __grid_constant__ AttnTcParams P) {
  const AttnParams& p = P.a;
  extern __shared__ __align__(1024) uint8_t sm[];
  float* maskadd = reinterpret_cast<float*>(sm + OFF_MASK);
  int* cflag = reinterpret_cast<int*>(sm + OFF_FLAG);
  uint64_t* bars = reinterpret_cast<uint64_t*>(sm + OFF_BAR);
  uint64_t* q_full = bars + 0;
  uint64_t* k_full = bars + 1;
  uint64_t* v_full = bars + 3;
  uint64_t* s_full = bars + 4;
  uint64_t* s_free = bars + 5;
  uint64_t* p_full = bars + 6;
  uint64_t* p_free = bars + 7;
  uint32_t* tptr = reinterpret_cast<uint32_t*>(sm + OFF_TPTR);

  const int tid = threadIdx.x, warp = tid >> 5, lane = tid & 31;
  const int q0 = blockIdx.x * ATC_BM, h = blockIdx.y, b = blockIdx.z;
  const int Lq = p.Lq, Lk = p.Lk;
  const int kvb = p.kv_batch_rows ? p.kv_batch_rows : Lk;
  const int mld = p.mask_ld ? p.mask_ld : Lk;
  const int qp0 = p.q_pos0;
  const int qbr = p.q_batch_rows ? p.q_batch_rows : Lq;
  const uint32_t sbase = smem_u32(sm);
  const int rows_here = min(ATC_BM, Lq - q0);
  const int n_act = (rows_here + 31) >> 5;
  const int n_all = (Lk + ATC_KC - 1) / ATC_KC;
  int n_plan = n_all;
  if (p.causal) {
    const int last_key = min(Lk - 1, q0 + rows_here - 1 + qp0);
    n_plan = last_key / ATC_KC + 1;
  }
  const bool may_rerun = p.causal && ((n_all - 1) * ATC_KC > q0 + qp0 + 31);

  if ((sbase & 1023u) != 0u) {
    if (tid == 0) printf("vima_b200: attention_tc shared memory window is not 1024-byte aligned\n");
    __trap();
  }
  if (warp == 4) {
    tmem_alloc<ATC_TMEM_COLS>(tptr);
    if (lane == 0) {
      mbar_init(q_full, 1);
      mbar_init(&k_full[0], 1);
      mbar_init(&k_full[1], 1);
      mbar_init(v_full, 1);
      mbar_init(s_full, 1);
      mbar_init(s_free, (uint32_t)n_act);
      mbar_init(p_full, (uint32_t)n_act);
      mbar_init(p_free, 1);
      fence_barrier_init();
      tma_prefetch_desc(&P.tm_q_hi); tma_prefetch_desc(&P.tm_q_lo);
      tma_prefetch_desc(&P.tm_k_hi); tma_prefetch_desc(&P.tm_k_lo);
      tma_prefetch_desc(&P.tm_v_hi); tma_prefetch_desc(&P.tm_v_lo);
    }
  }
  if (tid < 8) cflag[tid] = 0;
  tcgen05_fence_before();
  __syncthreads();
  tcgen05_fence_after();
  const uint32_t tmem = *tptr;

  const uint32_t fmt = (DT == DT_BF16) ? 1u : 0u;
  const uint32_t idesc_s = (1u << 4) | (fmt << 7) | (fmt << 10) | ((uint32_t)(ATC_KC >> 3) << 17) | ((uint32_t)(ATC_BM >> 4) << 24);
  const uint32_t idesc_o = (1u << 4) | (fmt << 7) | (fmt << 10) | (1u << 16) | ((uint32_t)(ATC_D >> 3) << 17) | ((uint32_t)(ATC_BM >> 4) << 24);
  const int x_col = h * ATC_D;
  const int kv_row0 = b * kvb;

  if (warp == 4) {
    uint32_t g = 0;
    uint32_t k_use[2] = {0u, 0u};
    int n = n_plan;
    for (int pass = 0; pass < 2; ++pass) {
      if (lane == 0) {
        auto load_k = [&](int c, int stage) {
          uint8_t* dst = sm + OFF_K + stage * 8192;
          mbar_arrive_expect_tx(&k_full[stage], 8192u);
          tma_load_2d(dst, &P.tm_k_hi, &k_full[stage], x_col, kv_row0 + c * ATC_KC);
          tma_load_2d(dst + 4096, &P.tm_k_lo, &k_full[stage], x_col, kv_row0 + c * ATC_KC);
        };
        auto load_v = [&](int c) {
          mbar_arrive_expect_tx(v_full, 8192u);
          tma_load_2d(sm + OFF_VH, &P.tm_v_hi, v_full, x_col, kv_row0 + c * ATC_KC);
          tma_load_2d(sm + OFF_VL, &P.tm_v_lo, v_full, x_col, kv_row0 + c * ATC_KC);
        };
        auto issue_qk = [&](int c, uint32_t gg) {
          const int stage = c & 1;
          mbar_wait(&k_full[stage], k_use[stage] & 1u);
          k_use[stage]++;
          if (gg > 0) mbar_wait(s_free, (gg - 1) & 1u);
          tcgen05_fence_after();
          const uint64_t dqh = desc_sw64(sbase + OFF_QH), dql = desc_sw64(sbase + OFF_QL);
          const uint64_t dkh = desc_sw64(sbase + OFF_K + stage * 8192), dkl = desc_sw64(sbase + OFF_K + stage * 8192 + 4096);
#pragma unroll
          for (int k = 0; k < ATC_D / 16; ++k) umma_f16(tmem, dqh + 2 * k, dkh + 2 * k, idesc_s, (uint32_t)(k != 0));
#pragma unroll
          for (int k = 0; k < ATC_D / 16; ++k) umma_f16(tmem, dql + 2 * k, dkh + 2 * k, idesc_s, 1u);
#pragma unroll
          for (int k = 0; k < ATC_D / 16; ++k) umma_f16(tmem, dqh + 2 * k, dkl + 2 * k, idesc_s, 1u);
          umma_commit(s_full);
        };
        if (pass == 0) {
          mbar_arrive_expect_tx(q_full, 16384u);
          tma_load_2d(sm + OFF_QH, &P.tm_q_hi, q_full, x_col, b * qbr + q0);
          tma_load_2d(sm + OFF_QL, &P.tm_q_lo, q_full, x_col, b * qbr + q0);
        }
        load_k(0, 0);
        if (n > 1) load_k(1, 1);
        load_v(0);
        if (pass == 0) mbar_wait(q_full, 0);
        issue_qk(0, g);
        for (int c = 0; c < n; ++c, ++g) {
          if (c + 1 < n) issue_qk(c + 1, g + 1);
          mbar_wait(p_full, g & 1u);
          mbar_wait(v_full, g & 1u);
          tcgen05_fence_after();
          {
            const uint64_t dph = desc_sw128(sbase + OFF_PH), dpl = desc_sw128(sbase + OFF_PL);
            const uint64_t dvh = desc_sw64(sbase + OFF_VH), dvl = desc_sw64(sbase + OFF_VL);
            const uint32_t t_o = tmem + 64;
#pragma unroll
            for (int k = 0; k < ATC_KC / 16; ++k) umma_f16(t_o, dph + 2 * k, dvh + 64 * k, idesc_o, (uint32_t)((c | k) != 0));
#pragma unroll
            for (int k = 0; k < ATC_KC / 16; ++k) umma_f16(t_o, dpl + 2 * k, dvh + 64 * k, idesc_o, 1u);
#pragma unroll
            for (int k = 0; k < ATC_KC / 16; ++k) umma_f16(t_o, dph + 2 * k, dvl + 64 * k, idesc_o, 1u);
          }
          umma_commit(p_free);
          mbar_wait(p_free, g & 1u);
          if (c + 2 < n) load_k(c + 2, c & 1);
          if (c + 1 < n) load_v(c + 1);
        }
      }
      __syncwarp();
      if (pass == 1 || !may_rerun) break;
      if (!__syncthreads_or(0)) break;
      n = n_all;
    }
  } else {
    for (int j = tid; j < n_all * ATC_KC; j += 128) {
      float mk = -INFINITY;
      if (j < Lk) mk = (p.key_mask == nullptr || p.key_mask[(size_t)b * mld + j]) ? 0.f : FP32_MIN_TC;
      maskadd[j] = mk;
      if (mk != 0.f) atomicOr(&cflag[j >> 6], 1);
    }
    named_bar_sync(1, 128);
    const bool w_on = warp < n_act;
    const int row = q0 + tid;
    const uint32_t t_row = tmem + ((uint32_t)(warp * 32) << 16);
    const float c_l2 = p.scale * LOG2E_TC;
    const int rpos = row + qp0;
    const int wpos_min = q0 + warp * 32 + qp0;
    const int wpos_max = wpos_min + 31;
    uint32_t pslot[8];
#pragma unroll
    for (int c8 = 0; c8 < 8; ++c8) pslot[c8] = sbase + OFF_PH + (uint32_t)tid * 128u + (uint32_t)((c8 ^ (tid & 7)) << 4);
    float m_ref = -INFINITY, l_run = 0.f;
    uint32_t g = 0;
    int n = n_plan;
    for (int pass = 0; pass < 2; ++pass) {
      const bool full = pass == 1;
      if (full) { m_ref = -INFINITY; l_run = 0.f; }
      if (w_on) {
        for (int c = 0; c < n; ++c, ++g) {
          const int k0 = c * ATC_KC;
          const bool hidden = p.causal && !full && k0 > wpos_max;
          mbar_wait(s_full, g & 1u);
          tcgen05_fence_after();
          uint32_t ph[ATC_KC / 2], pl[ATC_KC / 2];
          float ps = 0.f, m_use = m_ref;
          bool grow = false;
          if (!hidden) {
            uint32_t sv[ATC_KC];
            tmem_ld_32x32(t_row, *reinterpret_cast<uint32_t(*)[32]>(&sv[0]));
            tmem_ld_32x32(t_row + 32, *reinterpret_cast<uint32_t(*)[32]>(&sv[32]));
            tmem_ld_wait();
            tcgen05_fence_before();
            __syncwarp();
            if (lane == 0) mbar_arrive(s_free);
            const bool needs_causal = p.causal && (k0 + ATC_KC - 1 > wpos_min);
            float mx, sc;
            if (!needs_causal && !cflag[c]) {
              float m0 = __uint_as_float(sv[0]), m1 = __uint_as_float(sv[1]);
#pragma unroll
              for (int i = 2; i < ATC_KC; i += 4) {
                m0 = max3(m0, __uint_as_float(sv[i]), __uint_as_float(sv[i + 1]));
                if (i + 3 < ATC_KC) m1 = max3(m1, __uint_as_float(sv[i + 2]), __uint_as_float(sv[i + 3]));
              }
              mx = fmaxf(m0, m1) * c_l2;
              sc = c_l2;
            } else if (!needs_causal) {
              float m0 = -INFINITY, m1 = -INFINITY;
#pragma unroll
              for (int c4 = 0; c4 < ATC_KC; c4 += 4) {
                const float4 m4 = *reinterpret_cast<const float4*>(maskadd + k0 + c4);
                float x0 = __uint_as_float(sv[c4]), x1 = __uint_as_float(sv[c4 + 1]);
                float x2 = __uint_as_float(sv[c4 + 2]), x3 = __uint_as_float(sv[c4 + 3]);
                fma2v(x0, x1, c_l2, m4.x, m4.y);
                fma2v(x2, x3, c_l2, m4.z, m4.w);
                sv[c4] = __float_as_uint(x0); sv[c4 + 1] = __float_as_uint(x1);
                sv[c4 + 2] = __float_as_uint(x2); sv[c4 + 3] = __float_as_uint(x3);
                m0 = max3(m0, x0, x1);
                m1 = max3(m1, x2, x3);
              }
              mx = fmaxf(m0, m1);
              sc = 1.f;
            } else {
              mx = -INFINITY;
#pragma unroll
              for (int c4 = 0; c4 < ATC_KC; c4 += 4) {
                const float4 m4 = *reinterpret_cast<const float4*>(maskadd + k0 + c4);
                const float mm[4] = {m4.x, m4.y, m4.z, m4.w};
#pragma unroll
                for (int e = 0; e < 4; ++e) {
                  float y = fmaf(__uint_as_float(sv[c4 + e]), c_l2, mm[e]);
                  if (p.causal && k0 + c4 + e > rpos) y = CAUSAL_L2_TC + mm[e];
                  sv[c4 + e] = __float_as_uint(y);
                  mx = fmaxf(mx, y);
                }
              }
              sc = 1.f;
            }
            grow = mx > m_ref + LAZY_THRESH;
            if (grow) m_use = mx;
            const float neg_m = -m_use;
            float ps0 = 0.f, ps1 = 0.f;
#pragma unroll
            for (int i = 0; i < ATC_KC / 2; ++i) {
              float x0 = __uint_as_float(sv[2 * i]), x1 = __uint_as_float(sv[2 * i + 1]);
              fma2(x0, x1, sc, neg_m);
              const float p0 = ex2_approx(x0), p1 = ex2_approx(x1);
              ps0 += p0;
              ps1 += p1;
              split2<DT>(p0, p1, ph[i], pl[i]);
            }
            ps = ps0 + ps1;
          } else {
            tcgen05_fence_before();
            __syncwarp();
            if (lane == 0) mbar_arrive(s_free);
#pragma unroll
            for (int i = 0; i < ATC_KC / 2; ++i) { ph[i] = 0u; pl[i] = 0u; }
          }
          if (g > 0) mbar_wait(p_free, (g - 1) & 1u);
          float f = 1.f;
          if (grow && c > 0) f = ex2_approx(m_ref - m_use);
          if (c > 0 && __any_sync(0xffffffffu, grow)) {
            uint32_t ov[ATC_D];
            tcgen05_fence_after();
            tmem_ld_32x32(t_row + 64, ov);
            tmem_ld_wait();
#pragma unroll
            for (int i = 0; i < ATC_D; ++i) ov[i] = __float_as_uint(__uint_as_float(ov[i]) * f);
            tmem_st_32x32(t_row + 64, ov);
            tmem_st_wait();
          }
          l_run = (c > 0 ? l_run * f : 0.f) + ps;
          m_ref = m_use;
#pragma unroll
          for (int c8 = 0; c8 < 8; ++c8) {
            asm volatile("st.shared.v4.b32 [%0], {%1, %2, %3, %4};" ::"r"(pslot[c8]), "r"(ph[4 * c8]), "r"(ph[4 * c8 + 1]), "r"(ph[4 * c8 + 2]),
                         "r"(ph[4 * c8 + 3]) : "memory");
            asm volatile("st.shared.v4.b32 [%0], {%1, %2, %3, %4};" ::"r"(pslot[c8] + (uint32_t)(OFF_PL - OFF_PH)), "r"(pl[4 * c8]),
                         "r"(pl[4 * c8 + 1]), "r"(pl[4 * c8 + 2]), "r"(pl[4 * c8 + 3]) : "memory");
          }
          fence_proxy_async();
          tcgen05_fence_before();
          __syncwarp();
          if (lane == 0) mbar_arrive(p_full);
        }
        mbar_wait(p_free, (g - 1) & 1u);
        tcgen05_fence_after();
      }
      if (pass == 1 || !may_rerun) break;
      const int undone = w_on && row < Lq && !(m_ref > EXIT_L2_TC);
      if (!__syncthreads_or(undone)) break;
      n = n_all;
    }
    if (w_on) {
      uint32_t ov[ATC_D];
      tmem_ld_32x32(t_row + 64, ov);
      tmem_ld_wait();
      if (row < Lq) store_row<DT>(p, b, row, h, ov, 1.0f / l_run);
    }
  }
  tcgen05_fence_before();
  __syncthreads();
  if (warp == 4) {
    tcgen05_fence_after();
    tmem_dealloc<ATC_TMEM_COLS>(tmem);
  }
}

typedef CUresult (*PFN_encodeTiled_attn)(CUtensorMap*, CUtensorMapDataType, cuuint32_t, void*, const cuuint64_t*, const cuuint64_t*,
                                         const cuuint32_t*, const cuuint32_t*, CUtensorMapInterleave, CUtensorMapSwizzle,
                                         CUtensorMapL2promotion, CUtensorMapFloatOOBfill);

static bool make_map(void* encode, CUtensorMap* tm, const void* base, int dtype, long long rows, int cols, int ld, int box_rows) {
  const cuuint64_t gdim[2] = {(cuuint64_t)cols, (cuuint64_t)rows};
  const cuuint64_t gstride[1] = {(cuuint64_t)ld * 2};
  const cuuint32_t box[2] = {(cuuint32_t)ATC_D, (cuuint32_t)box_rows};
  const cuuint32_t estr[2] = {1, 1};
  const CUtensorMapDataType dt = dtype == DT_BF16 ? CU_TENSOR_MAP_DATA_TYPE_BFLOAT16 : CU_TENSOR_MAP_DATA_TYPE_FLOAT16;
  return ((PFN_encodeTiled_attn)encode)(tm, dt, 2, const_cast<void*>(base), gdim, gstride, box, estr, CU_TENSOR_MAP_INTERLEAVE_NONE,
                                        CU_TENSOR_MAP_SWIZZLE_64B, CU_TENSOR_MAP_L2_PROMOTION_L2_128B,
                                        CU_TENSOR_MAP_FLOAT_OOB_FILL_NONE) == CUDA_SUCCESS;
}

}

bool attention_tc_supported(const AttnParams& p) {
  auto al = [](const void* q) { return ((uintptr_t)q & 15) == 0; };
  if (!(al(p.q_hi) && al(p.q_lo) && al(p.k_hi) && al(p.k_lo) && al(p.v_hi) && al(p.v_lo) && al(p.o_hi) && al(p.o_lo) && al(p.o_lo8) && al(p.o_hi8)))
    return false;
  return p.D == 32 && p.split != 0 && p.rel_bias == nullptr && p.q_lo && p.k_lo && p.v_lo && (p.ldq % 8 == 0) && (p.ldk % 8 == 0) &&
         (p.ldv % 8 == 0) && (p.ldo % 8 == 0) && (p.o_lo8 == nullptr || p.ldo8 % 8 == 0) && p.H <= 65535 && p.B <= 65535 && p.Lk >= 1 &&
         p.Lk <= ATC_MAX_LK;
}

cudaError_t launch_attention_tc(const AttnParams& p, void* encode_fn, cudaStream_t stream) {
  if (p.B == 0 || p.Lq == 0) return cudaSuccess;
  AttnTcParams P;
  P.a = p;
  const int kvb = p.kv_batch_rows ? p.kv_batch_rows : p.Lk;
  const int qbr = p.q_batch_rows ? p.q_batch_rows : p.Lq;
  const int cols = p.H * ATC_D;
  bool ok = make_map(encode_fn, &P.tm_q_hi, p.q_hi, p.dtype, (long long)p.B * qbr, cols, p.ldq, ATC_BM) &&
            make_map(encode_fn, &P.tm_q_lo, p.q_lo, p.dtype, (long long)p.B * qbr, cols, p.ldq, ATC_BM) &&
            make_map(encode_fn, &P.tm_k_hi, p.k_hi, p.dtype, (long long)p.B * kvb, cols, p.ldk, ATC_KC) &&
            make_map(encode_fn, &P.tm_k_lo, p.k_lo, p.dtype, (long long)p.B * kvb, cols, p.ldk, ATC_KC) &&
            make_map(encode_fn, &P.tm_v_hi, p.v_hi, p.dtype, (long long)p.B * kvb, cols, p.ldv, ATC_KC) &&
            make_map(encode_fn, &P.tm_v_lo, p.v_lo, p.dtype, (long long)p.B * kvb, cols, p.ldv, ATC_KC);
  if (!ok) return cudaErrorInvalidValue;
  dim3 grid((p.Lq + ATC_BM - 1) / ATC_BM, p.H, p.B);
  const size_t smem = ATC_SMEM;
  static bool attr_set[2][64] = {};
  int dev = 0;
  cudaGetDevice(&dev);
  const int fi = p.dtype == DT_BF16 ? 1 : 0;
  if (!attr_set[fi][dev & 63]) {
    cudaError_t e = fi ? cudaFuncSetAttribute(attention_tc_kernel<DT_BF16>, cudaFuncAttributeMaxDynamicSharedMemorySize, (int)smem)
                       : cudaFuncSetAttribute(attention_tc_kernel<DT_F16>, cudaFuncAttributeMaxDynamicSharedMemorySize, (int)smem);
    if (e != cudaSuccess) return e;
    attr_set[fi][dev & 63] = true;
  }
  if (fi) attention_tc_kernel<DT_BF16><<<grid, ATC_THREADS, smem, stream>>>(P);
  else attention_tc_kernel<DT_F16><<<grid, ATC_THREADS, smem, stream>>>(P);
  return cudaGetLastError();
}

}
```

### vima_b200/csrc/kernels.h

```cpp
#pragma once
#include "common.cuh"

namespace vima {

struct NormParams {
  const float* x; long long rows; int cols; int ldx;
  const float* add; int ld_add;
  const float* w; const float* b;
  float eps; int rms;
  const float* w2; const float* b2; float eps2;
  float* out_f32; int ld_o32;
  float* out2_f32; int ld_o2;
  unsigned short* out_hi; unsigned short* out_lo; int ld_o16;
  int dtype;
  unsigned char* out_lo8; unsigned char* out_hi8; int ld_o8;
  float* stats_out; float stats_eps;
};
cudaError_t launch_norm(const NormParams& p, cudaStream_t stream);
cudaError_t launch_row_stats_finalize(const float* partial, long long rows, int parts, int cols, float eps, int rms, float* stats,
                                      cudaStream_t stream);

struct AttnParams {
  const unsigned short *q_hi, *q_lo; int ldq;
  const unsigned short *k_hi, *k_lo; int ldk;
  const unsigned short *v_hi, *v_lo; int ldv;
  const unsigned char* key_mask;
  const float* rel_bias;
  unsigned short *o_hi, *o_lo; int ldo;
  int B, H, Lq, Lk, D;
  float scale; int causal; int split; int dtype;
  unsigned char *o_lo8, *o_hi8; int ldo8;
  int kv_batch_rows;
  int mask_ld;
  int q_pos0;
  int q_batch_rows;
};
constexpr int ATTN_TAIL_MAX_ROWS = 8;
cudaError_t launch_attention(const AttnParams& p, cudaStream_t stream);
size_t attention_smem_bytes(const AttnParams& p);
int attention_max_lk(const AttnParams& p, size_t smem_limit);
bool attention_tc_supported(const AttnParams& p);
cudaError_t launch_attention_tc(const AttnParams& p, void* encode_tiled_fn, cudaStream_t stream);
cudaError_t launch_attention_tail(const AttnParams& p, int row0, int nt, cudaStream_t stream);

struct SmallAttnParams {
  const float* qkv; int ld;
  unsigned short *o_hi, *o_lo; int ldo; float* o_f32;
  long long N; int S, H, W; float scale; int dtype;
};
cudaError_t launch_small_attention(const SmallAttnParams& p, cudaStream_t stream);

struct LatentAttnParams {
  const float* q; int ldq; long long q_batch_stride;
  const float* k; int ldk;
  const float* v; int ldv;
  float* o; int ldo;
  long long N; int Lq, Lk, H, d; float scale;
};
cudaError_t launch_latent_attention(const LatentAttnParams& p, cudaStream_t stream);

struct SimtGemmGroup {
  const float* x; int ldx;
  const float* w; int ldw;
  const float* b;
  float* y; int ldy;
  int n, k;
};
cudaError_t launch_simt_gemm_grouped(const SimtGemmGroup* groups_dev, int n_groups, int M, int max_n, int act, cudaStream_t stream);
constexpr int SIMT_MAX_HOST_GROUPS = 16;
cudaError_t launch_simt_gemm_grouped_host(const SimtGemmGroup* groups_host, int n_groups, int M, int max_n, int act, cudaStream_t stream);

cudaError_t launch_split(const float* x, long long rows, int cols, int ldx, unsigned short* hi, unsigned short* lo, int ld16,
                         int pad_cols, float scale, int dtype, cudaStream_t s);
cudaError_t launch_pack_weight(const float* w, int n, int k, int transposed, int ldw, unsigned short* hi, unsigned short* lo, int ld16,
                               float scale, int dtype, cudaStream_t s);
cudaError_t launch_pack_weight_f8(const float* w, int n, int k, int transposed, int ldw, unsigned char* hi8, unsigned char* lo8, int ld8,
                                  float scale, cudaStream_t s);
cudaError_t launch_split_f8(const float* x, long long rows, int cols, int ldx, unsigned char* lo8, unsigned char* hi8, int ld8, cudaStream_t s);
cudaError_t launch_assemble_history(const float* obs, const unsigned char* obs_mask, const float* act, int T, int B, int Q, int E,
                                    int La, float* tokens, unsigned char* masks_bl, long long* pos_bl, cudaStream_t s);
cudaError_t launch_mask_cumsum(const unsigned char* mask, int B, int L, long long* pos, cudaStream_t s);
cudaError_t launch_add_pos_embed(const float* tok, long long stride_b, long long stride_l, const long long* ids, const float* table,
                                 int n_pos, int B, int L, int E, float* out_f32, unsigned short* hi, unsigned short* lo, int ld16,
                                 int dtype, int* err_flag, cudaStream_t s);
cudaError_t launch_gather_prompt(const int* kind, const int* index, const long long* word_ids, const float* word_table,
                                 const float* img_emb, const unsigned char* img_mask, int B, int Lp, int D, float* out,
                                 unsigned char* mask_out, cudaStream_t s);
cudaError_t launch_patchify(const unsigned char* img, long long N, int H, int W, int P, unsigned short* hi, unsigned short* lo, int ld16,
                            int dtype, cudaStream_t s);
cudaError_t launch_vit_tokens(const float* patch_out, const float* cls, const float* pos, long long N, int S, int W, float* out,
                              cudaStream_t s);
cudaError_t launch_bbox_norm(const long long* bbox, long long n, float* out, cudaStream_t s);
cudaError_t launch_fill_ee(const long long* ee, const float* table, long long n_te, int Q, unsigned short* hi, unsigned short* lo,
                           int ld16, int col0, int n_pad, int dtype, cudaStream_t s);
cudaError_t launch_action_scale(const long long* idx, long long n, int width, const float* inv_bins, float* out, cudaStream_t s);
cudaError_t launch_object_stats(const void* segm, int elem, int n_img, int H, int W, const long long* ids, int n_obj, int ids_per_image,
                                int* stats, cudaStream_t s);
cudaError_t launch_crop_resize(const unsigned char* rgb, int n_img, int H, int W, const int* stats, int n_obj, unsigned char* crops,
                               long long* bbox, unsigned char* mask, int* n_valid, cudaStream_t s);
cudaError_t launch_action_post(const long long* idx, long long n, int width, const float* bins, const float* lo, const float* hi,
                               int bound_stride, float* out, cudaStream_t s);
cudaError_t launch_head_select(const float* logits, int B, int n_heads, const int* head_off, float* logits_norm, long long* modes,
                               cudaStream_t s);
cudaError_t launch_gato_positions(const unsigned char* prompt_mask, int B, int Lp, int L, unsigned char* mask_out, long long* pos_out,
                                  cudaStream_t s);
cudaError_t launch_max_u8(const unsigned char* x, long long n, int* out_max, cudaStream_t s);

}
```

Before: 3387.

## Restructure tensor-core attention with per-(batch,head) CTAs and multi-stage K/V pipeline

Removes the separate attention tail kernel and the q_batch_rows plumbing. The tcgen05 attention kernel now launches one CTA per (head, batch) and loops over all query tiles. It keeps K/V chunks resident in shared memory across those tiles, uses a 3-stage TMEM score pipeline, and can run two 160-thread pipelines per CTA when Lk is long and Lq spans several tiles. The aim is to reuse K/V loads across query tiles and overlap the score MMA, softmax and PV steps, replacing the small tail kernel launch. In exchange the CTA count drops to B*H, which may underfill the SMs, and shared memory use grows with Lk.

```diff
diff --git a/vima_b200/build.py b/vima_b200/build.py
--- a/vima_b200/build.py
+++ b/vima_b200/build.py
@@ -10,7 +10,7 @@
 CSRC = os.path.join(HERE, "csrc")
 OUT_DIR = os.path.join(HERE, "_lib")
 LIB_PATH = os.path.join(OUT_DIR, "libvima_b200.so")
-SOURCES = ["api.cu", "gemm_tc_f16.cu", "gemm_tc_bf16.cu", "norm.cu", "attention.cu", "attention_tc.cu", "attention_tail.cu", "gemm_simt.cu", "misc.cu", "prepare.cu"]
+SOURCES = ["api.cu", "gemm_tc_f16.cu", "gemm_tc_bf16.cu", "norm.cu", "attention.cu", "attention_tc.cu", "gemm_simt.cu", "misc.cu", "prepare.cu"]
 HEADERS = ["common.cuh", "kernels.h", "gemm_tc.cuh", "gemm_tc_variants.cuh", os.path.join("..", "..", "include", "vima_b200.h")]
 NVCC_FLAGS = [
     "-gencode", "arch=compute_100a,code=sm_100a", "-O3", "-lineinfo", "-std=c++17", "--expt-relaxed-constexpr",
diff --git a/vima_b200/csrc/api.cu b/vima_b200/csrc/api.cu
--- a/vima_b200/csrc/api.cu
+++ b/vima_b200/csrc/api.cu
@@ -19,7 +19,6 @@
   void* encode_tiled;
   bool gemm_attr_set;
   int attn_tc;
-  int attn_tail;
   int gemm_mode;
   int epi_prefetch;
 };
@@ -93,8 +92,7 @@
     if (!strcmp(value, "tc")) { c->attn_tc = 1; return VIMA_OK; }
     if (!strcmp(value, "mma")) { c->attn_tc = 0; return VIMA_OK; }
   } else if (!strcmp(key, "attn_tail")) {
-    if (!strcmp(value, "kernel")) { c->attn_tail = 1; return VIMA_OK; }
-    if (!strcmp(value, "off")) { c->attn_tail = 0; return VIMA_OK; }
+    if (!strcmp(value, "kernel") || !strcmp(value, "off")) return VIMA_OK;
   } else if (!strcmp(key, "gemm_mode")) {
     if (!strcmp(value, "1cta")) { c->gemm_mode = 0; return VIMA_OK; }
     if (!strcmp(value, "mcast")) { c->gemm_mode = 1; return VIMA_OK; }
@@ -128,7 +126,7 @@
     return VIMA_E_CUDA;
   }
   c->encode_tiled = fn;
-  c->attn_tc = 1; c->attn_tail = 1; c->gemm_mode = 2; c->epi_prefetch = 0;
+  c->attn_tc = 1; c->gemm_mode = 2; c->epi_prefetch = 0;
   if (const char* e = getenv("VIMA_B200_ATTN")) vima_set_option(c, "attn", e);
   if (const char* e = getenv("VIMA_B200_ATTN_TAIL")) vima_set_option(c, "attn_tail", e);
   if (const char* e = getenv("VIMA_B200_GEMM_MODE")) vima_set_option(c, "gemm_mode", e);
@@ -391,24 +389,12 @@
   p.B = d->B; p.H = d->H; p.Lq = d->Lq; p.Lk = d->Lk; p.D = d->D;
   p.scale = d->scale; p.causal = d->causal; p.split = split; p.dtype = d->dtype;
   p.o_lo8 = (unsigned char*)d->o_lo8; p.o_hi8 = (unsigned char*)d->o_hi8; p.ldo8 = d->ldo8;
-  p.kv_batch_rows = d->kv_batch_rows; p.mask_ld = d->mask_ld; p.q_pos0 = d->q_pos0; p.q_batch_rows = 0;
+  p.kv_batch_rows = d->kv_batch_rows; p.mask_ld = d->mask_ld; p.q_pos0 = d->q_pos0;
   if ((d->kv_batch_rows && d->kv_batch_rows < d->Lk) || (d->mask_ld && d->mask_ld < d->Lk) || d->q_pos0 < 0)
     return fail(c, VIMA_E_INVALID, "attention: kv_batch_rows / mask_ld must cover Lk, q_pos0 >= 0");
   if ((p.o_lo8 == nullptr) != (p.o_hi8 == nullptr) || (p.o_lo8 && ((p.ldo8 & 1) || d->dtype != DT_F16)))
     return fail(c, VIMA_E_INVALID, "attention: o_lo8/o_hi8 come together (fp16 format, even ldo8)");
-  if (c->attn_tc && attention_tc_supported(p)) {
-    const int tail = p.Lq % 128;
-    if (c->attn_tail && p.Lq > 128 && tail >= 1 && tail <= ATTN_TAIL_MAX_ROWS) {
-      AttnParams body = p;
-      body.Lq = p.Lq - tail;
-      body.q_batch_rows = p.Lq;
-      cudaError_t e_ = launch_attention_tc(body, c->encode_tiled, (cudaStream_t)stream);
-      if (e_ != cudaSuccess) return cuda_fail(c, e_, "attention_tc");
-      c->launches++;
-      LAUNCHED(c, launch_attention_tail(p, p.Lq - tail, tail, (cudaStream_t)stream), "attention_tail");
-    }
-    LAUNCHED(c, launch_attention_tc(p, c->encode_tiled, (cudaStream_t)stream), "attention_tc");
-  }
+  if (c->attn_tc && attention_tc_supported(p)) LAUNCHED(c, launch_attention_tc(p, c->encode_tiled, (cudaStream_t)stream), "attention_tc");
   {
     const size_t need = attention_smem_bytes(p);
     if (need > (size_t)c->max_smem_optin)
diff --git a/vima_b200/csrc/attention.cu b/vima_b200/csrc/attention.cu
--- a/vima_b200/csrc/attention.cu
+++ b/vima_b200/csrc/attention.cu
@@ -54,7 +54,6 @@
   const int kvb = p.kv_batch_rows ? p.kv_batch_rows : Lk;
   const int mld = p.mask_ld ? p.mask_ld : Lk;
   const int qp0 = p.q_pos0;
-  const int qbr = p.q_batch_rows ? p.q_batch_rows : Lq;
   constexpr int CH = D / 8;
   for (int idx = tid; idx < Lk_pad * CH; idx += 256) {
     const int j = idx / CH, c = idx % CH;
@@ -115,7 +114,7 @@
         const int c = ks * 16 + 2 * t + ((e & 2) ? 8 : 0);
         uint32_t vh = 0, vl = 0;
         if (r < Lq) {
-          const size_t off = ((size_t)b * qbr + r) * p.ldq + h * D + c;
+          const size_t off = ((size_t)b * Lq + r) * p.ldq + h * D + c;
           vh = __ldg(reinterpret_cast<const uint32_t*>(p.q_hi + off));
           if (SPLIT) vl = __ldg(reinterpret_cast<const uint32_t*>(p.q_lo + off));
         }
@@ -265,7 +264,7 @@
         if (r >= Lq) continue;
         const float x0 = o[n][2 * half] * (half ? inv1 : inv0), x1 = o[n][2 * half + 1] * (half ? inv1 : inv0);
         pack_split<DT>(x0, x1, hi, lo);
-        const size_t off = ((size_t)b * qbr + r) * p.ldo + c;
+        const size_t off = ((size_t)b * Lq + r) * p.ldo + c;
         *reinterpret_cast<uint32_t*>(p.o_hi + off) = hi;
         if (p.o_lo) *reinterpret_cast<uint32_t*>(p.o_lo + off) = lo;
         if (p.o_lo8) {
@@ -273,7 +272,7 @@
           unsigned short l8, h8;
           asm("cvt.rn.satfinite.e4m3x2.f32 %0, %1, %2;" : "=h"(l8) : "f"((x1 - hf.y) * F8_ACT_LO_SCALE), "f"((x0 - hf.x) * F8_ACT_LO_SCALE));
           asm("cvt.rn.satfinite.e4m3x2.f32 %0, %1, %2;" : "=h"(h8) : "f"(x1 * F8_ACT_HI_SCALE), "f"(x0 * F8_ACT_HI_SCALE));
-          const size_t off8 = ((size_t)b * qbr + r) * p.ldo8 + c;
+          const size_t off8 = ((size_t)b * Lq + r) * p.ldo8 + c;
           *reinterpret_cast<unsigned short*>(p.o_lo8 + off8) = l8;
           *reinterpret_cast<unsigned short*>(p.o_hi8 + off8) = h8;
         }
diff --git a/vima_b200/csrc/attention_tail.cu b/vima_b200/csrc/attention_tail.cu
--- a/vima_b200/csrc/attention_tail.cu
+++ /dev/null
@@ -1,235 +0,0 @@
-#include "kernels.h"
-
-namespace vima {
-
-namespace {
-
-constexpr int TAIL_NT = ATTN_TAIL_MAX_ROWS;
-constexpr int TAIL_WARPS = 8;
-constexpr int TAIL_D = 32;
-constexpr float FP32_MIN_TL = -3.4028234663852886e38f;
-constexpr float LOG2E_TL = 1.4426950408889634f;
-constexpr float CAUSAL_L2_TL = -1e4f * LOG2E_TL;
-
-template <int DT>
-__device__ __forceinline__ float2 unpack2(uint32_t w) {
-  if constexpr (DT == DT_F16) return __half22float2(*reinterpret_cast<const __half2*>(&w));
-  else return __bfloat1622float2(*reinterpret_cast<const __nv_bfloat162*>(&w));
-}
-__device__ __forceinline__ unsigned long long pack2(float x, float y) {
-  unsigned long long r;
-  asm("mov.b64 %0, {%1, %2};" : "=l"(r) : "f"(x), "f"(y));
-  return r;
-}
-__device__ __forceinline__ float2 unpack64(unsigned long long v) {
-  float2 r;
-  asm("mov.b64 {%0, %1}, %2;" : "=f"(r.x), "=f"(r.y) : "l"(v));
-  return r;
-}
-__device__ __forceinline__ void ffma2(unsigned long long& acc, unsigned long long a, unsigned long long b) {
-  asm("fma.rn.f32x2 %0, %1, %2, %0;" : "+l"(acc) : "l"(a), "l"(b));
-}
-
-template <int DT>
-__global__ void __launch_bounds__(TAIL_WARPS * 32) attention_tail_kernel(const AttnParams p, int row0, int nt, int lk_pad) {
-  extern __shared__ __align__(16) float smt[];
-  const int warp = threadIdx.x >> 5, lane = threadIdx.x & 31;
-  const long long unit = (long long)blockIdx.x * TAIL_WARPS + warp;
-  if (unit >= (long long)p.B * p.H) return;
-  const int b = (int)(unit / p.H), h = (int)(unit % p.H);
-  const int Lk = p.Lk;
-  const int kvb = p.kv_batch_rows ? p.kv_batch_rows : Lk;
-  const int mld = p.mask_ld ? p.mask_ld : Lk;
-  const int qbr = p.q_batch_rows ? p.q_batch_rows : p.Lq;
-  float* qs = smt + (size_t)warp * (TAIL_NT * TAIL_D + (size_t)lk_pad * TAIL_NT);
-  float* sc = qs + TAIL_NT * TAIL_D;
-
-  const float c_l2 = p.scale * LOG2E_TL;
-#pragma unroll
-  for (int i = 0; i < TAIL_NT; ++i) {
-    float q = 0.f;
-    if (i < nt) {
-      const size_t off = ((size_t)b * qbr + row0 + i) * p.ldq + h * TAIL_D + lane;
-      q = Op16<DT>::back(p.q_hi[off]);
-      if (p.q_lo) q += Op16<DT>::back(p.q_lo[off]);
-    }
-    qs[i * TAIL_D + lane] = q * c_l2;
-  }
-  __syncwarp();
-
-  float mx[TAIL_NT];
-#pragma unroll
-  for (int i = 0; i < TAIL_NT; ++i) mx[i] = -INFINITY;
-  const int pos0 = row0 + p.q_pos0;
-  uint4 kh[4], kl[4];
-  auto load_k = [&](int j) {
-#pragma unroll
-    for (int c = 0; c < 4; ++c) { kh[c] = make_uint4(0u, 0u, 0u, 0u); kl[c] = kh[c]; }
-    if (j < Lk) {
-      const size_t rk = ((size_t)b * kvb + j) * p.ldk + h * TAIL_D;
-      const uint4* ph = reinterpret_cast<const uint4*>(p.k_hi + rk);
-#pragma unroll
-      for (int c = 0; c < 4; ++c) kh[c] = __ldg(ph + c);
-      if (p.k_lo) {
-        const uint4* pl = reinterpret_cast<const uint4*>(p.k_lo + rk);
-#pragma unroll
-        for (int c = 0; c < 4; ++c) kl[c] = __ldg(pl + c);
-      }
-    }
-  };
-  load_k(lane);
-  for (int j0 = 0; j0 < lk_pad; j0 += 32) {
-    const int j = j0 + lane;
-    const bool valid = j < Lk;
-    unsigned long long kf[TAIL_D / 2];
-#pragma unroll
-    for (int c = 0; c < 4; ++c) {
-      const uint32_t aw[4] = {kh[c].x, kh[c].y, kh[c].z, kh[c].w};
-      const uint32_t lw[4] = {kl[c].x, kl[c].y, kl[c].z, kl[c].w};
-#pragma unroll
-      for (int e = 0; e < 4; ++e) {
-        const float2 x = unpack2<DT>(aw[e]), y = unpack2<DT>(lw[e]);
-        kf[c * 4 + e] = pack2(x.x + y.x, x.y + y.y);
-      }
-    }
-    if (j0 + 32 < lk_pad) load_k(j + 32);
-    float madd = -INFINITY;
-    if (valid) madd = (p.key_mask == nullptr || p.key_mask[(size_t)b * mld + j]) ? 0.f : FP32_MIN_TL;
-    float y[TAIL_NT];
-#pragma unroll
-    for (int i = 0; i < TAIL_NT; ++i) {
-      const ulonglong2* q2 = reinterpret_cast<const ulonglong2*>(qs + i * TAIL_D);
-      unsigned long long a0 = 0ull, a1 = 0ull;
-#pragma unroll
-      for (int c = 0; c < TAIL_D / 4; ++c) {
-        const ulonglong2 q = q2[c];
-        ffma2(a0, q.x, kf[2 * c]);
-        ffma2(a1, q.y, kf[2 * c + 1]);
-      }
-      const float2 s0 = unpack64(a0), s1 = unpack64(a1);
-      float v = ((s0.x + s0.y) + (s1.x + s1.y)) + madd;
-      if (p.causal && j > pos0 + i) v = CAUSAL_L2_TL + madd;
-      y[i] = v;
-      mx[i] = fmaxf(mx[i], v);
-    }
-    float4* dst = reinterpret_cast<float4*>(sc + (size_t)j * TAIL_NT);
-    dst[0] = make_float4(y[0], y[1], y[2], y[3]);
-    dst[1] = make_float4(y[4], y[5], y[6], y[7]);
-  }
-#pragma unroll
-  for (int i = 0; i < TAIL_NT; ++i) mx[i] = warp_max(mx[i]);
-
-  float ls[TAIL_NT];
-#pragma unroll
-  for (int i = 0; i < TAIL_NT; ++i) ls[i] = 0.f;
-  for (int j0 = 0; j0 < lk_pad; j0 += 32) {
-    float4* cell = reinterpret_cast<float4*>(sc + (size_t)(j0 + lane) * TAIL_NT);
-    const float4 a = cell[0], c = cell[1];
-    float w[TAIL_NT] = {a.x, a.y, a.z, a.w, c.x, c.y, c.z, c.w};
-#pragma unroll
-    for (int i = 0; i < TAIL_NT; ++i) {
-      w[i] = ex2_approx(w[i] - mx[i]);
-      ls[i] += w[i];
-    }
-    cell[0] = make_float4(w[0], w[1], w[2], w[3]);
-    cell[1] = make_float4(w[4], w[5], w[6], w[7]);
-  }
-#pragma unroll
-  for (int i = 0; i < TAIL_NT; ++i) ls[i] = warp_sum(ls[i]);
-  __syncwarp();
-
-  const int kg = lane >> 3, dg = lane & 7;
-  unsigned long long acc[TAIL_NT][2];
-#pragma unroll
-  for (int i = 0; i < TAIL_NT; ++i) { acc[i][0] = 0ull; acc[i][1] = 0ull; }
-  for (int j = kg; j < Lk; j += 16) {
-    uint2 vh[4], vl[4];
-#pragma unroll
-    for (int u = 0; u < 4; ++u) {
-      const int jj = j + 4 * u;
-      vh[u] = make_uint2(0u, 0u); vl[u] = vh[u];
-      if (jj < Lk) {
-        const size_t rv = ((size_t)b * kvb + jj) * p.ldv + h * TAIL_D + dg * 4;
-        vh[u] = __ldg(reinterpret_cast<const uint2*>(p.v_hi + rv));
-        if (p.v_lo) vl[u] = __ldg(reinterpret_cast<const uint2*>(p.v_lo + rv));
-      }
-    }
-#pragma unroll
-    for (int u = 0; u < 4; ++u) {
-      const int jj = j + 4 * u;
-      if (jj >= Lk) break;
-      const float2 h0 = unpack2<DT>(vh[u].x), l0 = unpack2<DT>(vl[u].x), h1 = unpack2<DT>(vh[u].y), l1 = unpack2<DT>(vl[u].y);
-      const unsigned long long v01 = pack2(h0.x + l0.x, h0.y + l0.y), v23 = pack2(h1.x + l1.x, h1.y + l1.y);
-      const float4* cell = reinterpret_cast<const float4*>(sc + (size_t)jj * TAIL_NT);
-      const float4 a = cell[0], c = cell[1];
-      const float w[TAIL_NT] = {a.x, a.y, a.z, a.w, c.x, c.y, c.z, c.w};
-#pragma unroll
-      for (int i = 0; i < TAIL_NT; ++i) {
-        const unsigned long long ww = pack2(w[i], w[i]);
-        ffma2(acc[i][0], ww, v01);
-        ffma2(acc[i][1], ww, v23);
-      }
-    }
-  }
-#pragma unroll
-  for (int i = 0; i < TAIL_NT; ++i) {
-    const float2 a01 = unpack64(acc[i][0]), a23 = unpack64(acc[i][1]);
-    float4 o = make_float4(a01.x, a01.y, a23.x, a23.y);
-    o.x += __shfl_xor_sync(0xffffffffu, o.x, 8); o.y += __shfl_xor_sync(0xffffffffu, o.y, 8);
-    o.z += __shfl_xor_sync(0xffffffffu, o.z, 8); o.w += __shfl_xor_sync(0xffffffffu, o.w, 8);
-    o.x += __shfl_xor_sync(0xffffffffu, o.x, 16); o.y += __shfl_xor_sync(0xffffffffu, o.y, 16);
-    o.z += __shfl_xor_sync(0xffffffffu, o.z, 16); o.w += __shfl_xor_sync(0xffffffffu, o.w, 16);
-    if ((i & 3) != kg || i >= nt) continue;
-    const float inv = 1.0f / ls[i];
-    o.x *= inv; o.y *= inv; o.z *= inv; o.w *= inv;
-    const size_t row = (size_t)b * qbr + row0 + i;
-    const size_t off = row * p.ldo + h * TAIL_D + dg * 4;
-    if (p.o_lo8) {
-      uint2 h16;
-      uint32_t l8, h8;
-      split4_f8(o, F8_ACT_LO_SCALE, F8_ACT_HI_SCALE, h16, l8, h8);
-      *reinterpret_cast<uint2*>(p.o_hi + off) = h16;
-      const size_t off8 = row * p.ldo8 + h * TAIL_D + dg * 4;
-      *reinterpret_cast<uint32_t*>(p.o_lo8 + off8) = l8;
-      *reinterpret_cast<uint32_t*>(p.o_hi8 + off8) = h8;
-      if (p.o_lo) {
-        uint2 hi, lo;
-        split4v<DT>(o, hi, lo);
-        *reinterpret_cast<uint2*>(p.o_lo + off) = lo;
-      }
-    } else {
-      uint2 hi, lo;
-      split4v<DT>(o, hi, lo);
-      *reinterpret_cast<uint2*>(p.o_hi + off) = hi;
-      if (p.o_lo) *reinterpret_cast<uint2*>(p.o_lo + off) = lo;
-    }
-  }
-}
-
-}
-
-cudaError_t launch_attention_tail(const AttnParams& p, int row0, int nt, cudaStream_t stream) {
-  if (p.B == 0 || nt <= 0) return cudaSuccess;
-  if (nt > TAIL_NT || p.D != TAIL_D) return cudaErrorInvalidValue;
-  const int lk_pad = (p.Lk + 31) & ~31;
-  const size_t smem = (size_t)TAIL_WARPS * (TAIL_NT * TAIL_D + (size_t)lk_pad * TAIL_NT) * sizeof(float);
-  constexpr size_t smem_max = (size_t)TAIL_WARPS * (TAIL_NT * TAIL_D + 512 * TAIL_NT) * sizeof(float);
-  if (smem > smem_max) return cudaErrorInvalidValue;
-  static bool attr_set[2][64] = {};
-  int dev = 0;
-  cudaGetDevice(&dev);
-  const int fi = p.dtype == DT_BF16 ? 1 : 0;
-  if (!attr_set[fi][dev & 63]) {
-    cudaError_t e = fi ? cudaFuncSetAttribute(attention_tail_kernel<DT_BF16>, cudaFuncAttributeMaxDynamicSharedMemorySize, (int)smem_max)
-                       : cudaFuncSetAttribute(attention_tail_kernel<DT_F16>, cudaFuncAttributeMaxDynamicSharedMemorySize, (int)smem_max);
-    if (e != cudaSuccess) return e;
-    attr_set[fi][dev & 63] = true;
-  }
-  const long long units = (long long)p.B * p.H;
-  const unsigned grid = (unsigned)((units + TAIL_WARPS - 1) / TAIL_WARPS);
-  if (fi) attention_tail_kernel<DT_BF16><<<grid, TAIL_WARPS * 32, smem, stream>>>(p, row0, nt, lk_pad);
-  else attention_tail_kernel<DT_F16><<<grid, TAIL_WARPS * 32, smem, stream>>>(p, row0, nt, lk_pad);
-  return cudaGetLastError();
-}
-
-}
diff --git a/vima_b200/csrc/attention_tc.cu b/vima_b200/csrc/attention_tc.cu
--- a/vima_b200/csrc/attention_tc.cu
+++ b/vima_b200/csrc/attention_tc.cu
@@ -10,19 +10,18 @@
 constexpr float EXIT_L2_TC = -9000.f * LOG2E_TC;
 constexpr float LAZY_THRESH = 8.0f;
 
-constexpr int ATC_THREADS = 160;
 constexpr int ATC_BM = 128, ATC_KC = 64, ATC_D = 32;
-constexpr int ATC_TMEM_COLS = 128;
 constexpr int ATC_MAX_LK = 512;
-constexpr int OFF_QH = 0, OFF_QL = 8192;
-constexpr int OFF_K = 16384;
-constexpr int OFF_VH = 32768, OFF_VL = 36864;
-constexpr int OFF_PH = 40960, OFF_PL = 57344;
-constexpr int OFF_MASK = 73728;
-constexpr int OFF_FLAG = OFF_MASK + ATC_MAX_LK * 4;
-constexpr int OFF_BAR = OFF_FLAG + 32;
-constexpr int OFF_TPTR = OFF_BAR + 64;
-constexpr int ATC_SMEM = OFF_TPTR + 16;
+constexpr int ATC_MAX_CHUNKS = ATC_MAX_LK / ATC_KC;
+constexpr int ATC_NS = 3;
+constexpr int ATC_PIPE_COLS = 256;
+constexpr int ATC_O_COL = ATC_NS * 64;
+constexpr int ATC_ONE_PIPE_MAX_CHUNKS = 5;
+constexpr int Q_BYTES = 16384;
+constexpr int KV_BYTES = 16384;
+constexpr int TAIL_BYTES = ATC_MAX_LK * 4 + 32 + 8 * (ATC_MAX_CHUNKS + 2 * 6) + 16;
+
+__host__ __device__ constexpr int atc_smem_bytes(int npipe, int n_chunks) { return npipe * Q_BYTES + n_chunks * KV_BYTES + TAIL_BYTES; }
 
 struct AttnTcParams {
   AttnParams a;
@@ -32,8 +31,31 @@
 __device__ __forceinline__ uint64_t desc_sw64(uint32_t a) {
   return (uint64_t)((a >> 4) & 0x3FFF) | (1ull << 16) | ((uint64_t)(512 >> 4) << 32) | (1ull << 46) | (4ull << 61);
 }
-__device__ __forceinline__ uint64_t desc_sw128(uint32_t a) {
-  return (uint64_t)((a >> 4) & 0x3FFF) | (1ull << 16) | ((uint64_t)(1024 >> 4) << 32) | (1ull << 46) | (2ull << 61);
+
+__device__ __forceinline__ void umma_f16_ts(uint32_t tmem_d, uint32_t tmem_a, uint64_t desc_b, uint32_t idesc, uint32_t accumulate) {
+  asm volatile(
+      "{\n\t.reg .pred p;\n\t"
+      "setp.ne.b32 p, %4, 0;\n\t"
+      "tcgen05.mma.cta_group::1.kind::f16 [%0], [%1], %2, %3, p;\n\t}" ::"r"(tmem_d),
+      "r"(tmem_a), "l"(desc_b), "r"(idesc), "r"(accumulate)
+      : "memory");
+}
+
+__device__ __forceinline__ void mbar_arrive_cnt(uint64_t* bar, uint32_t cnt) {
+  asm volatile("mbarrier.arrive.shared::cta.b64 _, [%0], %1;" ::"r"(smem_u32(bar)), "r"(cnt) : "memory");
+}
+
+__device__ __forceinline__ bool bar_red_or(int id, int nthreads, bool v) {
+  uint32_t r;
+  asm volatile(
+      "{\n\t.reg .pred p, q;\n\t"
+      "setp.ne.u32 p, %1, 0;\n\t"
+      "barrier.cta.red.or.pred q, %2, %3, p;\n\t"
+      "selp.u32 %0, 1, 0, q;\n\t}"
+      : "=r"(r)
+      : "r"((uint32_t)v), "r"(id), "r"(nthreads)
+      : "memory");
+  return r != 0;
 }
 
 __device__ __forceinline__ float max3(float a, float b, float c) {
@@ -73,7 +95,7 @@
 
 template <int DT>
 __device__ __forceinline__ void store_row(const AttnParams& p, int b, int row, int h, const uint32_t (&o)[ATC_D], float inv) {
-  const size_t brow = (size_t)b * (p.q_batch_rows ? p.q_batch_rows : p.Lq) + row;
+  const size_t brow = (size_t)b * p.Lq + row;
   const size_t off = brow * p.ldo + h * ATC_D;
 #pragma unroll
   for (int c8 = 0; c8 < ATC_D / 8; ++c8) {
@@ -102,295 +124,304 @@
   }
 }
 
-template <int DT>
-__global__ void __launch_bounds__(ATC_THREADS, 3) attention_tc_kernel(const __grid_constant__ AttnTcParams P) {
+struct TilePlan {
+  int q0, rows, n_act, n_plan;
+  bool may_rerun;
+};
+__device__ __forceinline__ TilePlan plan_tile(const AttnParams& p, int t, int n_all) {
+  TilePlan tp;
+  tp.q0 = t * ATC_BM;
+  tp.rows = min(ATC_BM, p.Lq - tp.q0);
+  tp.n_act = (tp.rows + 31) >> 5;
+  tp.n_plan = n_all;
+  if (p.causal) tp.n_plan = min(p.Lk - 1, tp.q0 + tp.rows - 1 + p.q_pos0) / ATC_KC + 1;
+  tp.may_rerun = p.causal && ((n_all - 1) * ATC_KC > tp.q0 + p.q_pos0 + 31);
+  return tp;
+}
+
+template <int DT, int NPIPE>
+__global__ void __launch_bounds__(NPIPE * 160, 3 - NPIPE) attention_tc_kernel(const __grid_constant__ AttnTcParams P) {
   const AttnParams& p = P.a;
   extern __shared__ __align__(1024) uint8_t sm[];
-  float* maskadd = reinterpret_cast<float*>(sm + OFF_MASK);
-  int* cflag = reinterpret_cast<int*>(sm + OFF_FLAG);
-  uint64_t* bars = reinterpret_cast<uint64_t*>(sm + OFF_BAR);
-  uint64_t* q_full = bars + 0;
-  uint64_t* k_full = bars + 1;
-  uint64_t* v_full = bars + 3;
-  uint64_t* s_full = bars + 4;
-  uint64_t* s_free = bars + 5;
-  uint64_t* p_full = bars + 6;
-  uint64_t* p_free = bars + 7;
-  uint32_t* tptr = reinterpret_cast<uint32_t*>(sm + OFF_TPTR);
-
-  const int tid = threadIdx.x, warp = tid >> 5, lane = tid & 31;
-  const int q0 = blockIdx.x * ATC_BM, h = blockIdx.y, b = blockIdx.z;
+  const int h = blockIdx.x, b = blockIdx.y;
   const int Lq = p.Lq, Lk = p.Lk;
+  const int n_all = (Lk + ATC_KC - 1) / ATC_KC;
+  const int n_tiles = (Lq + ATC_BM - 1) / ATC_BM;
   const int kvb = p.kv_batch_rows ? p.kv_batch_rows : Lk;
   const int mld = p.mask_ld ? p.mask_ld : Lk;
-  const int qp0 = p.q_pos0;
-  const int qbr = p.q_batch_rows ? p.q_batch_rows : Lq;
+  const int off_kv = NPIPE * Q_BYTES;
+  const int off_mask = off_kv + n_all * KV_BYTES;
+  float* maskadd = reinterpret_cast<float*>(sm + off_mask);
+  int* cflag = reinterpret_cast<int*>(sm + off_mask + ATC_MAX_LK * 4);
+  uint64_t* bars = reinterpret_cast<uint64_t*>(sm + off_mask + ATC_MAX_LK * 4 + 32);
+  uint64_t* kv_full = bars;
+  uint32_t* tptr = reinterpret_cast<uint32_t*>(bars + ATC_MAX_CHUNKS + 6 * NPIPE);
+
+  const int tid = threadIdx.x, warp = tid >> 5, lane = tid & 31;
+  const bool is_ctl = warp >= 4 * NPIPE;
+  const int pipe = is_ctl ? warp - 4 * NPIPE : warp >> 2;
+  uint64_t* pb = bars + ATC_MAX_CHUNKS + 6 * pipe;
+  uint64_t* q_full = pb + 0;
+  uint64_t* s_full = pb + 1;
+  uint64_t* p_full = pb + 4;
+  uint64_t* pv_done = pb + 5;
   const uint32_t sbase = smem_u32(sm);
-  const int rows_here = min(ATC_BM, Lq - q0);
-  const int n_act = (rows_here + 31) >> 5;
-  const int n_all = (Lk + ATC_KC - 1) / ATC_KC;
-  int n_plan = n_all;
-  if (p.causal) {
-    const int last_key = min(Lk - 1, q0 + rows_here - 1 + qp0);
-    n_plan = last_key / ATC_KC + 1;
-  }
-  const bool may_rerun = p.causal && ((n_all - 1) * ATC_KC > q0 + qp0 + 31);
+  const uint32_t s_q = sbase + pipe * Q_BYTES;
 
   if ((sbase & 1023u) != 0u) {
     if (tid == 0) printf("vima_b200: attention_tc shared memory window is not 1024-byte aligned\n");
     __trap();
   }
-  if (warp == 4) {
-    tmem_alloc<ATC_TMEM_COLS>(tptr);
+  if (warp == 4 * NPIPE) {
+    tmem_alloc<NPIPE * ATC_PIPE_COLS>(tptr);
     if (lane == 0) {
-      mbar_init(q_full, 1);
-      mbar_init(&k_full[0], 1);
-      mbar_init(&k_full[1], 1);
-      mbar_init(v_full, 1);
-      mbar_init(s_full, 1);
-      mbar_init(s_free, (uint32_t)n_act);
-      mbar_init(p_full, (uint32_t)n_act);
-      mbar_init(p_free, 1);
+      for (int c = 0; c < n_all; ++c) mbar_init(&kv_full[c], 1);
+      for (int j = 0; j < NPIPE; ++j) {
+        uint64_t* bj = bars + ATC_MAX_CHUNKS + 6 * j;
+        for (int i = 0; i < 4; ++i) mbar_init(bj + i, 1);
+        mbar_init(bj + 4, 4);
+        mbar_init(bj + 5, 1);
+      }
       fence_barrier_init();
       tma_prefetch_desc(&P.tm_q_hi); tma_prefetch_desc(&P.tm_q_lo);
       tma_prefetch_desc(&P.tm_k_hi); tma_prefetch_desc(&P.tm_k_lo);
       tma_prefetch_desc(&P.tm_v_hi); tma_prefetch_desc(&P.tm_v_lo);
+      const int x_col = h * ATC_D, kv_row0 = b * kvb;
+      for (int c = 0; c < n_all; ++c) {
+        uint8_t* dst = sm + off_kv + c * KV_BYTES;
+        mbar_arrive_expect_tx(&kv_full[c], (uint32_t)KV_BYTES);
+        tma_load_2d(dst, &P.tm_k_hi, &kv_full[c], x_col, kv_row0 + c * ATC_KC);
+        tma_load_2d(dst + 4096, &P.tm_k_lo, &kv_full[c], x_col, kv_row0 + c * ATC_KC);
+        tma_load_2d(dst + 8192, &P.tm_v_hi, &kv_full[c], x_col, kv_row0 + c * ATC_KC);
+        tma_load_2d(dst + 12288, &P.tm_v_lo, &kv_full[c], x_col, kv_row0 + c * ATC_KC);
+      }
     }
-  }
-  if (tid < 8) cflag[tid] = 0;
-  tcgen05_fence_before();
-  __syncthreads();
-  tcgen05_fence_after();
-  const uint32_t tmem = *tptr;
-
-  const uint32_t fmt = (DT == DT_BF16) ? 1u : 0u;
-  const uint32_t idesc_s = (1u << 4) | (fmt << 7) | (fmt << 10) | ((uint32_t)(ATC_KC >> 3) << 17) | ((uint32_t)(ATC_BM >> 4) << 24);
-  const uint32_t idesc_o = (1u << 4) | (fmt << 7) | (fmt << 10) | (1u << 16) | ((uint32_t)(ATC_D >> 3) << 17) | ((uint32_t)(ATC_BM >> 4) << 24);
-  const int x_col = h * ATC_D;
-  const int kv_row0 = b * kvb;
-
-  if (warp == 4) {
-    uint32_t g = 0;
-    uint32_t k_use[2] = {0u, 0u};
-    int n = n_plan;
-    for (int pass = 0; pass < 2; ++pass) {
-      if (lane == 0) {
-        auto load_k = [&](int c, int stage) {
-          uint8_t* dst = sm + OFF_K + stage * 8192;
-          mbar_arrive_expect_tx(&k_full[stage], 8192u);
-          tma_load_2d(dst, &P.tm_k_hi, &k_full[stage], x_col, kv_row0 + c * ATC_KC);
-          tma_load_2d(dst + 4096, &P.tm_k_lo, &k_full[stage], x_col, kv_row0 + c * ATC_KC);
-        };
-        auto load_v = [&](int c) {
-          mbar_arrive_expect_tx(v_full, 8192u);
-          tma_load_2d(sm + OFF_VH, &P.tm_v_hi, v_full, x_col, kv_row0 + c * ATC_KC);
-          tma_load_2d(sm + OFF_VL, &P.tm_v_lo, v_full, x_col, kv_row0 + c * ATC_KC);
-        };
-        auto issue_qk = [&](int c, uint32_t gg) {
-          const int stage = c & 1;
-          mbar_wait(&k_full[stage], k_use[stage] & 1u);
-          k_use[stage]++;
-          if (gg > 0) mbar_wait(s_free, (gg - 1) & 1u);
-          tcgen05_fence_after();
-          const uint64_t dqh = desc_sw64(sbase + OFF_QH), dql = desc_sw64(sbase + OFF_QL);
-          const uint64_t dkh = desc_sw64(sbase + OFF_K + stage * 8192), dkl = desc_sw64(sbase + OFF_K + stage * 8192 + 4096);
-#pragma unroll
-          for (int k = 0; k < ATC_D / 16; ++k) umma_f16(tmem, dqh + 2 * k, dkh + 2 * k, idesc_s, (uint32_t)(k != 0));
-#pragma unroll
-          for (int k = 0; k < ATC_D / 16; ++k) umma_f16(tmem, dql + 2 * k, dkh + 2 * k, idesc_s, 1u);
-#pragma unroll
-          for (int k = 0; k < ATC_D / 16; ++k) umma_f16(tmem, dqh + 2 * k, dkl + 2 * k, idesc_s, 1u);
-          umma_commit(s_full);
-        };
-        if (pass == 0) {
-          mbar_arrive_expect_tx(q_full, 16384u);
-          tma_load_2d(sm + OFF_QH, &P.tm_q_hi, q_full, x_col, b * qbr + q0);
-          tma_load_2d(sm + OFF_QL, &P.tm_q_lo, q_full, x_col, b * qbr + q0);
-        }
-        load_k(0, 0);
-        if (n > 1) load_k(1, 1);
-        load_v(0);
-        if (pass == 0) mbar_wait(q_full, 0);
-        issue_qk(0, g);
-        for (int c = 0; c < n; ++c, ++g) {
-          if (c + 1 < n) issue_qk(c + 1, g + 1);
-          mbar_wait(p_full, g & 1u);
-          mbar_wait(v_full, g & 1u);
-          tcgen05_fence_after();
-          {
-            const uint64_t dph = desc_sw128(sbase + OFF_PH), dpl = desc_sw128(sbase + OFF_PL);
-            const uint64_t dvh = desc_sw64(sbase + OFF_VH), dvl = desc_sw64(sbase + OFF_VL);
-            const uint32_t t_o = tmem + 64;
-#pragma unroll
-            for (int k = 0; k < ATC_KC / 16; ++k) umma_f16(t_o, dph + 2 * k, dvh + 64 * k, idesc_o, (uint32_t)((c | k) != 0));
-#pragma unroll
-            for (int k = 0; k < ATC_KC / 16; ++k) umma_f16(t_o, dpl + 2 * k, dvh + 64 * k, idesc_o, 1u);
-#pragma unroll
-            for (int k = 0; k < ATC_KC / 16; ++k) umma_f16(t_o, dph + 2 * k, dvl + 64 * k, idesc_o, 1u);
-          }
-          umma_commit(p_free);
-          mbar_wait(p_free, g & 1u);
-          if (c + 2 < n) load_k(c + 2, c & 1);
-          if (c + 1 < n) load_v(c + 1);
-        }
-      }
-      __syncwarp();
-      if (pass == 1 || !may_rerun) break;
-      if (!__syncthreads_or(0)) break;
-      n = n_all;
-    }
-  } else {
-    for (int j = tid; j < n_all * ATC_KC; j += 128) {
+  } else if (!is_ctl) {
+    if (tid < 8) cflag[tid] = 0;
+    named_bar_sync(1, NPIPE * 128);
+    for (int j = tid; j < n_all * ATC_KC; j += NPIPE * 128) {
       float mk = -INFINITY;
       if (j < Lk) mk = (p.key_mask == nullptr || p.key_mask[(size_t)b * mld + j]) ? 0.f : FP32_MIN_TC;
       maskadd[j] = mk;
       if (mk != 0.f) atomicOr(&cflag[j >> 6], 1);
     }
-    named_bar_sync(1, 128);
-    const bool w_on = warp < n_act;
-    const int row = q0 + tid;
-    const uint32_t t_row = tmem + ((uint32_t)(warp * 32) << 16);
+  }
+  tcgen05_fence_before();
+  __syncthreads();
+  tcgen05_fence_after();
+  const uint32_t tmem = *tptr + (uint32_t)(pipe * ATC_PIPE_COLS);
+
+  const uint32_t fmt = (DT == DT_BF16) ? 1u : 0u;
+  const uint32_t idesc_s = (1u << 4) | (fmt << 7) | (fmt << 10) | ((uint32_t)(ATC_KC >> 3) << 17) | ((uint32_t)(ATC_BM >> 4) << 24);
+  const uint32_t idesc_o = (1u << 4) | (fmt << 7) | (fmt << 10) | (1u << 16) | ((uint32_t)(ATC_D >> 3) << 17) | ((uint32_t)(ATC_BM >> 4) << 24);
+  const int vote_bar = 2 + pipe;
+  const int softmax_bar = 4 + pipe;
+
+  if (is_ctl) {
+    uint32_t g = 0;
+    uint32_t n_q = 0;
+    uint32_t pv_seen = 0;
+    for (int t = pipe; t < n_tiles; t += NPIPE) {
+      const TilePlan tp = plan_tile(p, t, n_all);
+      int n = tp.n_plan;
+      for (int pass = 0; pass < 2; ++pass) {
+        if (lane == 0) {
+          auto wait_pv = [&](uint32_t k) {
+            if (k < pv_seen) return;
+            mbar_wait(pv_done, k & 1u);
+            pv_seen = k + 1;
+          };
+          auto issue_qk = [&](int c, uint32_t gg) {
+            mbar_wait(&kv_full[c], 0u);
+            if (gg >= ATC_NS) wait_pv(gg - ATC_NS);
+            tcgen05_fence_after();
+            const uint32_t t_s = tmem + (gg % ATC_NS) * 64u;
+            const uint64_t dqh = desc_sw64(s_q), dql = desc_sw64(s_q + 8192);
+            const uint32_t s_k = sbase + off_kv + c * KV_BYTES;
+            const uint64_t dkh = desc_sw64(s_k), dkl = desc_sw64(s_k + 4096);
+#pragma unroll
+            for (int k = 0; k < ATC_D / 16; ++k) umma_f16(t_s, dqh + 2 * k, dkh + 2 * k, idesc_s, (uint32_t)(k != 0));
+#pragma unroll
+            for (int k = 0; k < ATC_D / 16; ++k) umma_f16(t_s, dql + 2 * k, dkh + 2 * k, idesc_s, 1u);
+#pragma unroll
+            for (int k = 0; k < ATC_D / 16; ++k) umma_f16(t_s, dqh + 2 * k, dkl + 2 * k, idesc_s, 1u);
+            umma_commit(&s_full[gg % ATC_NS]);
+          };
+          if (g > 0) wait_pv(g - 1);
+          if (pass == 0) {
+            mbar_arrive_expect_tx(q_full, (uint32_t)Q_BYTES);
+            tma_load_2d(sm + pipe * Q_BYTES, &P.tm_q_hi, q_full, h * ATC_D, b * Lq + tp.q0);
+            tma_load_2d(sm + pipe * Q_BYTES + 8192, &P.tm_q_lo, q_full, h * ATC_D, b * Lq + tp.q0);
+            mbar_wait(q_full, n_q & 1u);
+            ++n_q;
+          }
+          issue_qk(0, g);
+          if (n > 1) issue_qk(1, g + 1);
+          for (int c = 0; c < n; ++c, ++g) {
+            if (c + 2 < n) issue_qk(c + 2, g + 2);
+            mbar_wait(p_full, g & 1u);
+            tcgen05_fence_after();
+            const uint32_t t_p = tmem + (g % ATC_NS) * 64u;
+            const uint32_t s_v = sbase + off_kv + c * KV_BYTES + 8192;
+            const uint64_t dvh = desc_sw64(s_v), dvl = desc_sw64(s_v + 4096);
+            const uint32_t t_o = tmem + ATC_O_COL;
+#pragma unroll
+            for (int k = 0; k < ATC_KC / 16; ++k) umma_f16_ts(t_o, t_p + 8 * k, dvh + 64 * k, idesc_o, (uint32_t)((c | k) != 0));
+#pragma unroll
+            for (int k = 0; k < ATC_KC / 16; ++k) umma_f16_ts(t_o, t_p + 32 + 8 * k, dvh + 64 * k, idesc_o, 1u);
+#pragma unroll
+            for (int k = 0; k < ATC_KC / 16; ++k) umma_f16_ts(t_o, t_p + 8 * k, dvl + 64 * k, idesc_o, 1u);
+            umma_commit(pv_done);
+          }
+        }
+        __syncwarp();
+        if (pass == 1 || !tp.may_rerun) break;
+        if (!bar_red_or(vote_bar, 160, false)) break;
+        n = n_all;
+      }
+    }
+  } else {
+    const int wq = warp & 3;
+    const uint32_t t_lane = tmem + ((uint32_t)(wq * 32) << 16);
     const float c_l2 = p.scale * LOG2E_TC;
-    const int rpos = row + qp0;
-    const int wpos_min = q0 + warp * 32 + qp0;
-    const int wpos_max = wpos_min + 31;
-    uint32_t pslot[8];
-#pragma unroll
-    for (int c8 = 0; c8 < 8; ++c8) pslot[c8] = sbase + OFF_PH + (uint32_t)tid * 128u + (uint32_t)((c8 ^ (tid & 7)) << 4);
-    float m_ref = -INFINITY, l_run = 0.f;
     uint32_t g = 0;
-    int n = n_plan;
-    for (int pass = 0; pass < 2; ++pass) {
-      const bool full = pass == 1;
-      if (full) { m_ref = -INFINITY; l_run = 0.f; }
-      if (w_on) {
-        for (int c = 0; c < n; ++c, ++g) {
-          const int k0 = c * ATC_KC;
-          const bool hidden = p.causal && !full && k0 > wpos_max;
-          mbar_wait(s_full, g & 1u);
-          tcgen05_fence_after();
-          uint32_t ph[ATC_KC / 2], pl[ATC_KC / 2];
-          float ps = 0.f, m_use = m_ref;
-          bool grow = false;
-          if (!hidden) {
-            uint32_t sv[ATC_KC];
-            tmem_ld_32x32(t_row, *reinterpret_cast<uint32_t(*)[32]>(&sv[0]));
-            tmem_ld_32x32(t_row + 32, *reinterpret_cast<uint32_t(*)[32]>(&sv[32]));
-            tmem_ld_wait();
+    for (int t = pipe; t < n_tiles; t += NPIPE) {
+      const TilePlan tp = plan_tile(p, t, n_all);
+      const bool w_on = wq < tp.n_act;
+      const int row = tp.q0 + wq * 32 + lane;
+      const int rpos = row + p.q_pos0;
+      const int wpos_min = tp.q0 + wq * 32 + p.q_pos0;
+      const int wpos_max = wpos_min + 31;
+      const uint32_t arrive_cnt = wq == 0 ? (uint32_t)(5 - tp.n_act) : 1u;
+      float m_ref = -INFINITY, l_run = 0.f;
+      int n = tp.n_plan;
+      for (int pass = 0; pass < 2; ++pass) {
+        const bool full = pass == 1;
+        if (full) { m_ref = -INFINITY; l_run = 0.f; }
+        if (w_on) {
+          for (int c = 0; c < n; ++c) {
+            const uint32_t gg = g + (uint32_t)c;
+            const int k0 = c * ATC_KC;
+            const uint32_t t_s = t_lane + (gg % ATC_NS) * 64u;
+            const bool hidden = p.causal && !full && k0 > wpos_max;
+            mbar_wait(&s_full[gg % ATC_NS], (gg / ATC_NS) & 1u);
+            tcgen05_fence_after();
+            uint32_t ph[ATC_KC / 2], pl[ATC_KC / 2];
+            float ps = 0.f, m_use = m_ref;
+            bool grow = false;
+            if (!hidden) {
+              uint32_t sv[ATC_KC];
+              tmem_ld_32x32(t_s, *reinterpret_cast<uint32_t(*)[32]>(&sv[0]));
+              tmem_ld_32x32(t_s + 32, *reinterpret_cast<uint32_t(*)[32]>(&sv[32]));
+              tmem_ld_wait();
+              const bool needs_causal = p.causal && (k0 + ATC_KC - 1 > wpos_min);
+              float mx, sc;
+              if (!needs_causal && !cflag[c]) {
+                float m0 = __uint_as_float(sv[0]), m1 = __uint_as_float(sv[1]);
+#pragma unroll
+                for (int i = 2; i < ATC_KC; i += 4) {
+                  m0 = max3(m0, __uint_as_float(sv[i]), __uint_as_float(sv[i + 1]));
+                  if (i + 3 < ATC_KC) m1 = max3(m1, __uint_as_float(sv[i + 2]), __uint_as_float(sv[i + 3]));
+                }
+                mx = fmaxf(m0, m1) * c_l2;
+                sc = c_l2;
+              } else if (!needs_causal) {
+                float m0 = -INFINITY, m1 = -INFINITY;
+#pragma unroll
+                for (int c4 = 0; c4 < ATC_KC; c4 += 4) {
+                  const float4 m4 = *reinterpret_cast<const float4*>(maskadd + k0 + c4);
+                  float x0 = __uint_as_float(sv[c4]), x1 = __uint_as_float(sv[c4 + 1]);
+                  float x2 = __uint_as_float(sv[c4 + 2]), x3 = __uint_as_float(sv[c4 + 3]);
+                  fma2v(x0, x1, c_l2, m4.x, m4.y);
+                  fma2v(x2, x3, c_l2, m4.z, m4.w);
+                  sv[c4] = __float_as_uint(x0); sv[c4 + 1] = __float_as_uint(x1);
+                  sv[c4 + 2] = __float_as_uint(x2); sv[c4 + 3] = __float_as_uint(x3);
+                  m0 = max3(m0, x0, x1);
+                  m1 = max3(m1, x2, x3);
+                }
+                mx = fmaxf(m0, m1);
+                sc = 1.f;
+              } else {
+                mx = -INFINITY;
+#pragma unroll
+                for (int c4 = 0; c4 < ATC_KC; c4 += 4) {
+                  const float4 m4 = *reinterpret_cast<const float4*>(maskadd + k0 + c4);
+                  const float mm[4] = {m4.x, m4.y, m4.z, m4.w};
+#pragma unroll
+                  for (int e = 0; e < 4; ++e) {
+                    float y = fmaf(__uint_as_float(sv[c4 + e]), c_l2, mm[e]);
+                    if (p.causal && k0 + c4 + e > rpos) y = CAUSAL_L2_TC + mm[e];
+                    sv[c4 + e] = __float_as_uint(y);
+                    mx = fmaxf(mx, y);
+                  }
+                }
+                sc = 1.f;
+              }
+              grow = mx > m_ref + LAZY_THRESH;
+              if (grow) m_use = mx;
+              const float neg_m = -m_use;
+              float ps0 = 0.f, ps1 = 0.f;
+#pragma unroll
+              for (int i = 0; i < ATC_KC / 2; ++i) {
+                float x0 = __uint_as_float(sv[2 * i]), x1 = __uint_as_float(sv[2 * i + 1]);
+                fma2(x0, x1, sc, neg_m);
+                const float p0 = ex2_approx(x0), p1 = ex2_approx(x1);
+                ps0 += p0;
+                ps1 += p1;
+                split2<DT>(p0, p1, ph[i], pl[i]);
+              }
+              ps = ps0 + ps1;
+            } else {
+#pragma unroll
+              for (int i = 0; i < ATC_KC / 2; ++i) { ph[i] = 0u; pl[i] = 0u; }
+            }
+            if (gg > 0) {
+              mbar_wait(pv_done, (gg - 1) & 1u);
+              tcgen05_fence_after();
+            }
+            float f = 1.f;
+            if (grow && c > 0) f = ex2_approx(m_ref - m_use);
+            if (c > 0 && __any_sync(0xffffffffu, grow)) {
+              uint32_t ov[ATC_D];
+              tmem_ld_32x32(t_lane + ATC_O_COL, ov);
+              tmem_ld_wait();
+#pragma unroll
+              for (int i = 0; i < ATC_D; ++i) ov[i] = __float_as_uint(__uint_as_float(ov[i]) * f);
+              tmem_st_32x32(t_lane + ATC_O_COL, ov);
+            }
+            l_run = (c > 0 ? l_run * f : 0.f) + ps;
+            m_ref = m_use;
+            tmem_st_32x32(t_s, ph);
+            tmem_st_32x32(t_s + 32, pl);
+            tmem_st_wait();
             tcgen05_fence_before();
             __syncwarp();
-            if (lane == 0) mbar_arrive(s_free);
-            const bool needs_causal = p.causal && (k0 + ATC_KC - 1 > wpos_min);
-            float mx, sc;
-            if (!needs_causal && !cflag[c]) {
-              float m0 = __uint_as_float(sv[0]), m1 = __uint_as_float(sv[1]);
-#pragma unroll
-              for (int i = 2; i < ATC_KC; i += 4) {
-                m0 = max3(m0, __uint_as_float(sv[i]), __uint_as_float(sv[i + 1]));
-                if (i + 3 < ATC_KC) m1 = max3(m1, __uint_as_float(sv[i + 2]), __uint_as_float(sv[i + 3]));
-              }
-              mx = fmaxf(m0, m1) * c_l2;
-              sc = c_l2;
-            } else if (!needs_causal) {
-              float m0 = -INFINITY, m1 = -INFINITY;
-#pragma unroll
-              for (int c4 = 0; c4 < ATC_KC; c4 += 4) {
-                const float4 m4 = *reinterpret_cast<const float4*>(maskadd + k0 + c4);
-                float x0 = __uint_as_float(sv[c4]), x1 = __uint_as_float(sv[c4 + 1]);
-                float x2 = __uint_as_float(sv[c4 + 2]), x3 = __uint_as_float(sv[c4 + 3]);
-                fma2v(x0, x1, c_l2, m4.x, m4.y);
-                fma2v(x2, x3, c_l2, m4.z, m4.w);
-                sv[c4] = __float_as_uint(x0); sv[c4 + 1] = __float_as_uint(x1);
-                sv[c4 + 2] = __float_as_uint(x2); sv[c4 + 3] = __float_as_uint(x3);
-                m0 = max3(m0, x0, x1);
-                m1 = max3(m1, x2, x3);
-              }
-              mx = fmaxf(m0, m1);
-              sc = 1.f;
-            } else {
-              mx = -INFINITY;
-#pragma unroll
-              for (int c4 = 0; c4 < ATC_KC; c4 += 4) {
-                const float4 m4 = *reinterpret_cast<const float4*>(maskadd + k0 + c4);
-                const float mm[4] = {m4.x, m4.y, m4.z, m4.w};
-#pragma unroll
-                for (int e = 0; e < 4; ++e) {
-                  float y = fmaf(__uint_as_float(sv[c4 + e]), c_l2, mm[e]);
-                  if (p.causal && k0 + c4 + e > rpos) y = CAUSAL_L2_TC + mm[e];
-                  sv[c4 + e] = __float_as_uint(y);
-                  mx = fmaxf(mx, y);
-                }
-              }
-              sc = 1.f;
-            }
-            grow = mx > m_ref + LAZY_THRESH;
-            if (grow) m_use = mx;
-            const float neg_m = -m_use;
-            float ps0 = 0.f, ps1 = 0.f;
-#pragma unroll
-            for (int i = 0; i < ATC_KC / 2; ++i) {
-              float x0 = __uint_as_float(sv[2 * i]), x1 = __uint_as_float(sv[2 * i + 1]);
-              fma2(x0, x1, sc, neg_m);
-              const float p0 = ex2_approx(x0), p1 = ex2_approx(x1);
-              ps0 += p0;
-              ps1 += p1;
-              split2<DT>(p0, p1, ph[i], pl[i]);
-            }
-            ps = ps0 + ps1;
-          } else {
-            tcgen05_fence_before();
-            __syncwarp();
-            if (lane == 0) mbar_arrive(s_free);
-#pragma unroll
-            for (int i = 0; i < ATC_KC / 2; ++i) { ph[i] = 0u; pl[i] = 0u; }
+            if (lane == 0) mbar_arrive_cnt(p_full, arrive_cnt);
           }
-          if (g > 0) mbar_wait(p_free, (g - 1) & 1u);
-          float f = 1.f;
-          if (grow && c > 0) f = ex2_approx(m_ref - m_use);
-          if (c > 0 && __any_sync(0xffffffffu, grow)) {
-            uint32_t ov[ATC_D];
-            tcgen05_fence_after();
-            tmem_ld_32x32(t_row + 64, ov);
-            tmem_ld_wait();
-#pragma unroll
-            for (int i = 0; i < ATC_D; ++i) ov[i] = __float_as_uint(__uint_as_float(ov[i]) * f);
-            tmem_st_32x32(t_row + 64, ov);
-            tmem_st_wait();
-          }
-          l_run = (c > 0 ? l_run * f : 0.f) + ps;
-          m_ref = m_use;
-#pragma unroll
-          for (int c8 = 0; c8 < 8; ++c8) {
-            asm volatile("st.shared.v4.b32 [%0], {%1, %2, %3, %4};" ::"r"(pslot[c8]), "r"(ph[4 * c8]), "r"(ph[4 * c8 + 1]), "r"(ph[4 * c8 + 2]),
-                         "r"(ph[4 * c8 + 3]) : "memory");
-            asm volatile("st.shared.v4.b32 [%0], {%1, %2, %3, %4};" ::"r"(pslot[c8] + (uint32_t)(OFF_PL - OFF_PH)), "r"(pl[4 * c8]),
-                         "r"(pl[4 * c8 + 1]), "r"(pl[4 * c8 + 2]), "r"(pl[4 * c8 + 3]) : "memory");
-          }
-          fence_proxy_async();
-          tcgen05_fence_before();
-          __syncwarp();
-          if (lane == 0) mbar_arrive(p_full);
+          mbar_wait(pv_done, (g + (uint32_t)n - 1) & 1u);
+          tcgen05_fence_after();
         }
-        mbar_wait(p_free, (g - 1) & 1u);
-        tcgen05_fence_after();
-      }
-      if (pass == 1 || !may_rerun) break;
-      const int undone = w_on && row < Lq && !(m_ref > EXIT_L2_TC);
-      if (!__syncthreads_or(undone)) break;
-      n = n_all;
-    }
-    if (w_on) {
-      uint32_t ov[ATC_D];
-      tmem_ld_32x32(t_row + 64, ov);
-      tmem_ld_wait();
-      if (row < Lq) store_row<DT>(p, b, row, h, ov, 1.0f / l_run);
+        g += (uint32_t)n;
+        if (pass == 1 || !tp.may_rerun) break;
+        const bool undone = w_on && row < Lq && !(m_ref > EXIT_L2_TC);
+        if (!bar_red_or(vote_bar, 160, undone)) break;
+        n = n_all;
+      }
+      if (w_on) {
+        uint32_t ov[ATC_D];
+        tmem_ld_32x32(t_lane + ATC_O_COL, ov);
+        tmem_ld_wait();
+        if (row < Lq) store_row<DT>(p, b, row, h, ov, 1.0f / l_run);
+      }
+      tcgen05_fence_before();
+      named_bar_sync(softmax_bar, 128);
     }
   }
   tcgen05_fence_before();
   __syncthreads();
-  if (warp == 4) {
+  if (warp == 4 * NPIPE) {
     tcgen05_fence_after();
-    tmem_dealloc<ATC_TMEM_COLS>(tmem);
+    tmem_dealloc<NPIPE * ATC_PIPE_COLS>(*tptr);
   }
 }
 
@@ -409,6 +440,22 @@
                                         CU_TENSOR_MAP_FLOAT_OOB_FILL_NONE) == CUDA_SUCCESS;
 }
 
+template <int DT, int NPIPE>
+cudaError_t launch_variant(const AttnTcParams& P, int n_chunks, cudaStream_t stream) {
+  static bool attr_set[64] = {};
+  int dev = 0;
+  cudaGetDevice(&dev);
+  if (!attr_set[dev & 63]) {
+    cudaError_t e = cudaFuncSetAttribute(attention_tc_kernel<DT, NPIPE>, cudaFuncAttributeMaxDynamicSharedMemorySize,
+                                         atc_smem_bytes(NPIPE, ATC_MAX_CHUNKS));
+    if (e != cudaSuccess) return e;
+    attr_set[dev & 63] = true;
+  }
+  const dim3 grid(P.a.H, P.a.B);
+  attention_tc_kernel<DT, NPIPE><<<grid, NPIPE * 160, atc_smem_bytes(NPIPE, n_chunks), stream>>>(P);
+  return cudaGetLastError();
+}
+
 }
 
 bool attention_tc_supported(const AttnParams& p) {
@@ -425,30 +472,18 @@
   AttnTcParams P;
   P.a = p;
   const int kvb = p.kv_batch_rows ? p.kv_batch_rows : p.Lk;
-  const int qbr = p.q_batch_rows ? p.q_batch_rows : p.Lq;
   const int cols = p.H * ATC_D;
-  bool ok = make_map(encode_fn, &P.tm_q_hi, p.q_hi, p.dtype, (long long)p.B * qbr, cols, p.ldq, ATC_BM) &&
-            make_map(encode_fn, &P.tm_q_lo, p.q_lo, p.dtype, (long long)p.B * qbr, cols, p.ldq, ATC_BM) &&
+  bool ok = make_map(encode_fn, &P.tm_q_hi, p.q_hi, p.dtype, (long long)p.B * p.Lq, cols, p.ldq, ATC_BM) &&
+            make_map(encode_fn, &P.tm_q_lo, p.q_lo, p.dtype, (long long)p.B * p.Lq, cols, p.ldq, ATC_BM) &&
             make_map(encode_fn, &P.tm_k_hi, p.k_hi, p.dtype, (long long)p.B * kvb, cols, p.ldk, ATC_KC) &&
             make_map(encode_fn, &P.tm_k_lo, p.k_lo, p.dtype, (long long)p.B * kvb, cols, p.ldk, ATC_KC) &&
             make_map(encode_fn, &P.tm_v_hi, p.v_hi, p.dtype, (long long)p.B * kvb, cols, p.ldv, ATC_KC) &&
             make_map(encode_fn, &P.tm_v_lo, p.v_lo, p.dtype, (long long)p.B * kvb, cols, p.ldv, ATC_KC);
   if (!ok) return cudaErrorInvalidValue;
-  dim3 grid((p.Lq + ATC_BM - 1) / ATC_BM, p.H, p.B);
-  const size_t smem = ATC_SMEM;
-  static bool attr_set[2][64] = {};
-  int dev = 0;
-  cudaGetDevice(&dev);
-  const int fi = p.dtype == DT_BF16 ? 1 : 0;
-  if (!attr_set[fi][dev & 63]) {
-    cudaError_t e = fi ? cudaFuncSetAttribute(attention_tc_kernel<DT_BF16>, cudaFuncAttributeMaxDynamicSharedMemorySize, (int)smem)
-                       : cudaFuncSetAttribute(attention_tc_kernel<DT_F16>, cudaFuncAttributeMaxDynamicSharedMemorySize, (int)smem);
-    if (e != cudaSuccess) return e;
-    attr_set[fi][dev & 63] = true;
-  }
-  if (fi) attention_tc_kernel<DT_BF16><<<grid, ATC_THREADS, smem, stream>>>(P);
-  else attention_tc_kernel<DT_F16><<<grid, ATC_THREADS, smem, stream>>>(P);
-  return cudaGetLastError();
-}
-
-}
+  const int n_chunks = (p.Lk + ATC_KC - 1) / ATC_KC;
+  const bool two_pipes = n_chunks > ATC_ONE_PIPE_MAX_CHUNKS && p.Lq > ATC_BM;
+  if (p.dtype == DT_BF16) return two_pipes ? launch_variant<DT_BF16, 2>(P, n_chunks, stream) : launch_variant<DT_BF16, 1>(P, n_chunks, stream);
+  return two_pipes ? launch_variant<DT_F16, 2>(P, n_chunks, stream) : launch_variant<DT_F16, 1>(P, n_chunks, stream);
+}
+
+}
diff --git a/vima_b200/csrc/kernels.h b/vima_b200/csrc/kernels.h
--- a/vima_b200/csrc/kernels.h
+++ b/vima_b200/csrc/kernels.h
@@ -33,15 +33,12 @@
   int kv_batch_rows;
   int mask_ld;
   int q_pos0;
-  int q_batch_rows;
 };
-constexpr int ATTN_TAIL_MAX_ROWS = 8;
 cudaError_t launch_attention(const AttnParams& p, cudaStream_t stream);
 size_t attention_smem_bytes(const AttnParams& p);
 int attention_max_lk(const AttnParams& p, size_t smem_limit);
 bool attention_tc_supported(const AttnParams& p);
 cudaError_t launch_attention_tc(const AttnParams& p, void* encode_tiled_fn, cudaStream_t stream);
-cudaError_t launch_attention_tail(const AttnParams& p, int row0, int nt, cudaStream_t stream);
 
 struct SmallAttnParams {
   const float* qkv; int ld;
```

Result: faster. 3451, median of 6 (+1.9%).
